# probsys/AutoGP.jl

Measured on AMD Instinct MI355X. Metric: particle_logpdf_evals_per_sec, higher is better.
Workload: dtype f64

## Files before the change

autogp.jl_amd/__init__.py:

```python
from .gp import (Node, LeafNode, BinaryOpNode, WhiteNoise, Constant, Linear, SquaredExponential,
                 GammaExponential, Periodic, Plus, Times, ChangePoint, unroll, encode, encode_batch, from_tuple,
                 split_kernel_sop, extract_kernel)
from .engine import (GPEngine, GPEngineMulti, shard_range, shard_plan, probe_lattice, logpdf_grad_batch_multi, predict_batch_multi, AGPError, PosDefException, load_library, LIB_PATH, EXPORTED_SYMBOLS,
                     compute_cov_matrix_vectorized, eval_cov, mvnormal_logpdf, MvNormal, quantile, infer_gp_sum, predict_proba,
                     predict_quantile, predict_quantile_multi, raw_components, predict_mvn_sum, predict_sum, predict_rand,
                     MixtureModel, predict_mvn, pack_series, series_call_args, SERIES_MAX_N)
from . import prior, schedule, dist, stream

__all__ = [n for n in dir() if not n.startswith("_")]
```

autogp.jl_amd/csrc/agp_common.hpp:

```cpp
#pragma once
#include <hip/hip_runtime.h>
#include <stdint.h>

namespace agp {

constexpr int NB = 128;
constexpr int NB2 = NB * NB;
constexpr int BS = 16;
constexpr int NSB = NB / BS;
constexpr int KB = 16;
constexpr int AGP_MAX_OPS_DEV = 256;
constexpr int LDS_STRIDE = 144;

enum : int { OP_WN = 0, OP_CONST = 1, OP_LIN = 2, OP_SE = 3, OP_GE = 4, OP_PER = 5,
             OP_PLUS = 6, OP_TIMES = 7, OP_CP = 8, OP_CP_SWAP = 9, OP_SEL = 10, OP_GE_TAB = 11,
             OP_LAG = 12 };
constexpr double LOGDT_ZERO = -1.0e8;

struct ProgHdr {
  int32_t op_off;
  int32_t prm_off;
  int32_t n_ops;
  int32_t n_cp;
  int32_t n_prm;
  int32_t flags;
  int32_t n_lag;
  int32_t lag_off;
};

struct LagTabHdr {
  int32_t op_off, n_ops, prm_off, pad_;
};

__host__ __device__ inline long long tile_off(int i, int j) {
  return ((long long)i * (i + 1) / 2 + j) * (long long)NB2;
}

typedef double d4 __attribute__((ext_vector_type(4)));
typedef double d2 __attribute__((ext_vector_type(2)));

}
```

autogp.jl_amd/csrc/agp_cov_kernel.hpp:

```cpp
#pragma once
#ifndef AGP_EXP_TABLE
#define AGP_EXP_TABLE 1
#endif
#include "agp_common.hpp"
#include "agp_args.hpp"
#include "agp_math.hpp"

namespace agp {

__device__ __forceinline__ int prm_count(int o) {
  return (o == OP_WN || o == OP_CONST || o == OP_SEL) ? 1 : (o == OP_SE || o == OP_CP || o == OP_CP_SWAP) ? 2
         : (o == OP_PLUS || o == OP_TIMES || o == OP_LAG) ? 0 : 3;
}

template <bool LAG = false, typename OpT>
__device__ __forceinline__ void cov_prologue(const double* __restrict__ tt, const uint8_t* __restrict__ code,
                                             int ti, int tj, const ProgHdr& h,
                                             const OpT* __restrict__ ops, const double* __restrict__ prm,
                                             double* tpt, double* sig, int tid,
                                             const double* __restrict__ lagtab = nullptr, int nt = 0,
                                             const int32_t* __restrict__ rank = nullptr, int lstride = 256, int* xrk = nullptr,
                                             bool copy_rank_tables = true, const CltArgs clt = CltArgs{}, int* cbl = nullptr) {
  const int g = (tid < NB) ? (ti * NB + tid) : (tj * NB + (tid - NB));
  const double tg = tt[g];
  if (LAG && h.n_lag > 0) {
    double* lag = sig + h.n_cp * 256;
    if (rank != nullptr) {
      if (clt.B != nullptr && copy_rank_tables) {
        const int odmin = clt.W > 0 ? (ti > tj ? (ti - tj) * NB - (NB - 1) : 0) : 0;
        const int woff = clt.W * odmin;
        for (int li = 0; li < h.n_lag; ++li) {
          const double* __restrict__ src = lagtab + (long long)(h.lag_off + li) * clt.gstride + woff;
          for (int i = tid; i < lstride; i += 256) lag[li * lstride + i] = src[i];
        }
        for (int i = tid; i < clt.nB; i += 256) cbl[i] = clt.B[odmin + i] - woff;
      } else {
        const double* __restrict__ src = lagtab + (long long)h.lag_off * lstride;
        if (copy_rank_tables)
          for (int i = tid; i < h.n_lag * lstride; i += 256) lag[i] = src[i];
      }
      xrk[tid] = rank[g];
    } else {
      const double* __restrict__ src = lagtab + ((long long)h.lag_off * nt + (ti - tj)) * 256 + tid;
      for (int li = 0; li < h.n_lag; ++li) lag[li * 256 + tid] = src[(long long)li * nt * 256];
    }
  }
  tpt[tid] = tg;
  __syncthreads();
  if (h.n_cp > 0) {
    const double t = tg;
    const int cd = code ? (int)code[g] : 0;
    int q = 0, c = 0;
    for (int ip = 0; ip < h.n_ops; ++ip) {
      const int o = __builtin_amdgcn_readfirstlane((int)ops[ip]);
      if (o == OP_CP || o == OP_CP_SWAP) {
        const double loc = prm[q], sc = prm[q + 1];
        sig[c * 256 + tid] = 0.5 * (1.0 + tanh((loc - t) / sc));
        ++c;
      } else if (o == OP_SEL) {
        const int id = (int)prm[q];
        sig[c * 256 + tid] = (cd == 0 || cd == id) ? 1.0 : 0.0;
        ++c;
      }
      q += prm_count(o);
    }
    __syncthreads();
  }
}

template <int E, int GEMODE>
__device__ __forceinline__ void eval_leaf(const int o, const double p0, const double p1, const double p2,
                                          const double* sg, const double* lg,
                                          const double (&tr)[E], const double (&tc)[E],
                                          const int (&ri)[E], const int (&ci)[E], const double (&lt)[E],
                                          const double* etab, double (&v)[E], const int* rk = nullptr, const int* cb = nullptr) {
  auto ex = [&](double x) { return (AGP_EXP_TABLE != 0) ? fm::exp_t(x, etab) : fm::exp_f(x); };
  if (o == OP_SEL) {
#pragma unroll
    for (int e = 0; e < E; ++e) v[e] = sg[ri[e]] * sg[ci[e]];
  } else if (o == OP_WN) {
#pragma unroll
    for (int e = 0; e < E; ++e) v[e] = (tr[e] == tc[e]) ? p0 : 0.0;
  } else if (o == OP_CONST) {
#pragma unroll
    for (int e = 0; e < E; ++e) v[e] = p0;
  } else if (o == OP_LIN) {
#pragma unroll
    for (int e = 0; e < E; ++e) v[e] = p1 + p2 * ((tr[e] - p0) * (tc[e] - p0));
  } else if ((GEMODE == 0 || GEMODE == 3) && (GEMODE == 3 || o == OP_LAG)) {
    if (cb != nullptr) {
#pragma unroll
      for (int e = 0; e < E; ++e) {
        const int d0 = rk[ri[e]] - rk[ci[e]], d = d0 < 0 ? -d0 : d0;
        v[e] = lg[(d & CLT_MASK) + cb[d >> CLT_SHIFT]];
      }
    } else if (rk != nullptr) {
#pragma unroll
      for (int e = 0; e < E; ++e) { const int d = rk[ri[e]] - rk[ci[e]]; v[e] = lg[d < 0 ? -d : d]; }
    } else {
      const double* lq_ = lg + (2 * NB - 1);
#pragma unroll
      for (int e = 0; e < E; ++e) v[e] = lq_[ri[e] - ci[e]];
    }
  } else if (GEMODE != 3) {
    double arg[E];
    const double amp = (o == OP_SE) ? p1 : p2;
    if (o == OP_SE) {
#pragma unroll
      for (int e = 0; e < E; ++e) {
        const double dx = tr[e] - tc[e];
        arg[e] = ((-0.5 * dx) * dx) * p0;
      }
    } else if (GEMODE != 2 && o == OP_GE) {
#pragma unroll
      for (int e = 0; e < E; ++e) arg[e] = -fm::pow_f(fabs(tr[e] - tc[e]) * p0, p1);
    } else if (GEMODE != 1 && (o == OP_GE_TAB || (GEMODE == 2 && o == OP_GE))) {
#pragma unroll
      for (int e = 0; e < E; ++e) arg[e] = -ex(p1 * (lt[e] - p0));
    } else {
#pragma unroll
      for (int e = 0; e < E; ++e) arg[e] = p0 * fm::sin2_f(p1 * fabs(tr[e] - tc[e]));
    }
#pragma unroll
    for (int e = 0; e < E; ++e) v[e] = amp * ex(arg[e]);
  }
}

template <int D, int E, int GEMODE = 0, typename OpT>
__device__ __forceinline__ void eval_program(const ProgHdr& h, const OpT* __restrict__ ops,
                                             const double* __restrict__ prm, const double* sig,
                                             const double (&tr)[E], const double (&tc)[E],
                                             const int (&ri)[E], const int (&ci)[E], const double (&lt)[E],
                                             double (&out)[E], const double* etab = nullptr, const double* lag = nullptr,
                                             const int* rk = nullptr, int lstride = 256, const int* cb = nullptr) {
  double st[D][E];
#pragma unroll
  for (int d = 0; d < D; ++d)
#pragma unroll
    for (int e = 0; e < E; ++e) st[d][e] = 0.0;

  int q = 0, cpi = 0, li = 0;
  for (int ip = 0; ip < h.n_ops; ++ip) {
    const int o = __builtin_amdgcn_readfirstlane((int)ops[ip]);
    if (o <= OP_PER || o >= OP_SEL) {
      const double p0 = prm[q], p1 = prm[q + 1], p2 = prm[q + 2];
      double v[E];
      eval_leaf<E, GEMODE>(o, p0, p1, p2, sig + cpi * 256, lag + li * lstride, tr, tc, ri, ci, lt, etab, v, rk, cb);
      if (o == OP_SEL) ++cpi;
      if (o == OP_LAG) ++li;
#pragma unroll
      for (int d = D - 1; d > 0; --d)
#pragma unroll
        for (int e = 0; e < E; ++e) st[d][e] = st[d - 1][e];
#pragma unroll
      for (int e = 0; e < E; ++e) st[0][e] = v[e];
    } else {
      if (o == OP_PLUS) {
#pragma unroll
        for (int e = 0; e < E; ++e) st[0][e] = st[1][e] + st[0][e];
      } else if (o == OP_TIMES) {
#pragma unroll
        for (int e = 0; e < E; ++e) st[0][e] = st[1][e] * st[0][e];
      } else {
        const double* sg = sig + cpi * 256;
#pragma unroll
        for (int e = 0; e < E; ++e) {
          const double si = sg[ri[e]];
          const double sj = sg[ci[e]];
          const double kl = (o == OP_CP) ? st[1][e] : st[0][e];
          const double kr = (o == OP_CP) ? st[0][e] : st[1][e];
          st[0][e] = (si * sj) * kl + ((1.0 - si) * (1.0 - sj)) * kr;
        }
        ++cpi;
      }
#pragma unroll
      for (int d = 1; d < D - 1; ++d)
#pragma unroll
        for (int e = 0; e < E; ++e) st[d][e] = st[d + 1][e];
    }
    q += prm_count(o);
  }
#pragma unroll
  for (int e = 0; e < E; ++e) out[e] = st[0][e];
}

__device__ __forceinline__ double cov_finalize(double v, int gi, int gj, int n1, int n1_pad, int m2, double noise) {
  const bool vi = (gi < n1) || (gi >= n1_pad && gi < n1_pad + m2);
  const bool vj = (gj < n1) || (gj >= n1_pad && gj < n1_pad + m2);
  double r = (vi && vj) ? v : 0.0;
  if (gi == gj) r = vi ? (r + noise) : 1.0;
  return r;
}
__device__ __forceinline__ double diag_noise(const double* noise, const double* noise_q, int p, int tk, int n1_pad) {
  const double* q = tk * NB < n1_pad ? noise : noise_q;
  return q != nullptr ? q[p] : 0.0;
}

#ifndef AGP_COV_E
#define AGP_COV_E 4
#endif
#ifndef AGP_COV_WGS
#define AGP_COV_WGS 4
#endif
template <int D>
__global__ __launch_bounds__(256, AGP_COV_WGS) void k_cov_tiles(CovArgs a) {
  constexpr int E = AGP_COV_E, CPP = E / 2;
  const int cpt = a.csplit == 4 ? 8 : 32;
  const int NPASS = cpt / CPP;
  extern __shared__ __attribute__((aligned(16))) double smem[];
  double* tpt = smem;
  double* sig = smem + 256;

  const int p = blockIdx.y + a.p_off;
  const int tix = blockIdx.x;
  int ti, tj;
  ti = (int)((sqrt(8.0 * (double)tix + 1.0) - 1.0) * 0.5);
  while (ti * (ti + 1) / 2 > tix) --ti;
  while ((ti + 1) * (ti + 2) / 2 <= tix) ++ti;
  tj = tix - ti * (ti + 1) / 2;
  if (a.i0 != nullptr && ti < a.i0[p]) return;
  if (a.skip_pred_offdiag && ti != tj && tj * NB >= a.n1_pad) return;
  if (a.pred_only && tj * NB < a.n1_pad) return;
  const int tid = threadIdx.x;
  const ProgHdr h = a.hdr[p];
  const uint8_t* __restrict__ ops = a.ops + h.op_off;
  const double* __restrict__ prm = a.prm + h.prm_off;
  const bool rankt = a.lagr != nullptr;
  const int lstride = rankt ? (a.clt.B != nullptr ? a.clt.gstride : a.lag_stride) : 256;
  int* xrk = reinterpret_cast<int*>(sig + h.n_cp * 256 + (rankt ? 0 : h.n_lag * 256));
  double* etab = reinterpret_cast<double*>(xrk) + (rankt ? 128 : 0);
  if (AGP_EXP_TABLE && tid < AGP_EXP_TAB_N) etab[tid] = fm::c_exp_tab[tid];
  cov_prologue<true>(a.tt, a.code, ti, tj, h, ops, prm, tpt, sig, tid, a.lagtab, a.nt, a.lagr, lstride, xrk, false);
  const double* lag = rankt ? a.lagtab + (long long)h.lag_off * lstride : sig + h.n_cp * 256;
  const int* rk = rankt ? xrk : nullptr;
  const int* cb = rankt ? a.clt.B : nullptr;

  const int rp = tid & 63;
  const int cb0 = a.csplit == 4 ? (int)blockIdx.z * 32 + (tid >> 6) * 8 : (tid >> 6) * 32;
  const int r0 = 2 * rp;
  const double tr0 = tpt[r0], tr1 = tpt[r0 + 1];
  const int gi0 = ti * NB + r0;
  const double noise = diag_noise(a.noise, a.noise_q, p, tj, a.n1_pad);
  double* __restrict__ T = a.A + (long long)(a.slot != nullptr ? a.slot[p] : p) * a.strideA + tile_off(ti, tj);

  const bool use_tab = (h.flags & 1) != 0;
  const double* __restrict__ ltile = a.logdt + tile_off(ti, tj);
  d2 ltn[CPP];
#pragma unroll
  for (int cc = 0; cc < CPP; ++cc) ltn[cc] = d2{0.0, 0.0};
  if (use_tab) {
#pragma unroll
    for (int cc = 0; cc < CPP; ++cc) ltn[cc] = *reinterpret_cast<const d2*>(ltile + (long long)(cb0 + cc) * NB + r0);
  }
  const bool one_node = h.n_ops == 1;
  const int op1 = one_node ? __builtin_amdgcn_readfirstlane((int)ops[0]) : -1;
  const double q0 = one_node ? prm[0] : 0.0, q1 = one_node ? prm[1] : 0.0, q2 = one_node ? prm[2] : 0.0;
  for (int pass = 0; pass < NPASS; ++pass) {
    const int c0 = cb0 + pass * CPP;
    double tr[E], tc[E], out[E], lt[E];
    int ri[E], ci[E];
#pragma unroll
    for (int cc = 0; cc < CPP; ++cc) { lt[2 * cc] = ltn[cc].x; lt[2 * cc + 1] = ltn[cc].y; }
    if (use_tab && pass + 1 < NPASS) {
#pragma unroll
      for (int cc = 0; cc < CPP; ++cc) ltn[cc] = *reinterpret_cast<const d2*>(ltile + (long long)(c0 + CPP + cc) * NB + r0);
    }
#pragma unroll
    for (int e = 0; e < E; ++e) {
      tr[e] = (e & 1) ? tr1 : tr0;
      tc[e] = tpt[NB + c0 + (e >> 1)];
      ri[e] = r0 + (e & 1);
      ci[e] = NB + c0 + (e >> 1);
    }
    if (one_node) eval_leaf<E, 0>(op1, q0, q1, q2, sig, lag, tr, tc, ri, ci, lt, etab, out, rk, cb);
    else eval_program<D, E, 0>(h, ops, prm, sig, tr, tc, ri, ci, lt, out, etab, lag, rk, lstride, cb);
#pragma unroll
    for (int cc = 0; cc < CPP; ++cc) {
      const int gj = tj * NB + c0 + cc;
      d2 o2;
      o2.x = cov_finalize(out[2 * cc], gi0, gj, a.n1, a.n1_pad, a.m2, noise);
      o2.y = cov_finalize(out[2 * cc + 1], gi0 + 1, gj, a.n1, a.n1_pad, a.m2, noise);
      *reinterpret_cast<d2*>(T + (long long)(c0 + cc) * NB + r0) = o2;
    }
  }
}

#ifdef AGP_KERNEL_TU_MAIN
__global__ __launch_bounds__(256) void k_lag_tables(LagArgs a) {
  const int t = blockIdx.y, bl = blockIdx.x, tid = threadIdx.x;
  __shared__ double etab[AGP_EXP_TAB_N];
  if (AGP_EXP_TABLE && tid < AGP_EXP_TAB_N) etab[tid] = fm::c_exp_tab[tid];
  __syncthreads();
  const LagTabHdr th = a.thdr[t];
  ProgHdr h = {};
  h.n_ops = th.n_ops;
  int g = a.full ? bl * 256 + tid : bl * NB + tid - (NB - 1);
  if (g < 0) g = -g;
  const bool live = a.full ? g < a.nt * NB : (tid < 2 * NB - 1 && g < a.nt * NB);
  const double tr[1] = {live ? a.tt[g] : 0.0}, tc[1] = {live ? a.tt[0] : 0.0}, lt[1] = {0.0};
  const int ri[1] = {0}, ci[1] = {NB};
  double out[1];
  eval_program<8, 1, 1>(h, a.tops + th.op_off, a.tprm + th.prm_off, nullptr, tr, tc, ri, ci, lt, out, etab);
  if (a.full) a.tab[(long long)t * a.stride + g] = out[0];
  else a.tab[((long long)t * a.nt + bl) * 256 + tid] = out[0];
}

__global__ __launch_bounds__(256) void k_logdt_tiles(const double* __restrict__ tt, double* __restrict__ T) {
  const int tix = blockIdx.x;
  int ti = (int)((sqrt(8.0 * (double)tix + 1.0) - 1.0) * 0.5);
  while (ti * (ti + 1) / 2 > tix) --ti;
  while ((ti + 1) * (ti + 2) / 2 <= tix) ++ti;
  const int tj = tix - ti * (ti + 1) / 2;
  double* __restrict__ out = T + tile_off(ti, tj);
  for (int e = threadIdx.x; e < NB2; e += 256) {
    const int r = e & (NB - 1), cidx = e >> 7;
    const double dt = fabs(tt[ti * NB + r] - tt[tj * NB + cidx]);
    out[e] = dt > 0.0 ? fm::log_f(dt) : LOGDT_ZERO;
  }
}

#endif

}
```

autogp.jl_amd/csrc/agp_engine.hip:

```cpp
#include "agp_host.hpp"

thread_local std::string g_err_noctx;

std::atomic<long long> HostProf::ns[HostProf::N];
std::atomic<long long> HostProf::cnt[HostProf::N];
const char* HostProf::names[HostProf::N] = {"coalesce: assemble", "dedup keys", "compile_batch", "grad classify + residency", "store lookup (grad)",
    "slot + buffers + staging", "launches (value)", "launches (grad)", "wait + copy back", "scatter results", "extend: keys + dedup",
    "extend: capacity + slots", "extend: compile", "extend: staging + launches", "extend: wait + register", "coalesce: hand back",
    "  of which: factor part", "  of which: gradient launches", "", "", "", "", "", ""};
int HostProf::enabled() {
  static int e = -1;
  if (e < 0) { const char* v = getenv("AGP_HOST_PROF"); e = (v && atoi(v) != 0) ? 1 : 0; }
  return e;
}
void HostProf::report() {
  if (enabled() <= 0) return;
  fprintf(stderr, "[AGP_HOST_PROF] stage                              calls     total ms    us / call\n");
  for (int i = 0; i < N; ++i) {
    const long long k = cnt[i].load(), t = ns[i].load();
    if (k > 0) fprintf(stderr, "[AGP_HOST_PROF] %-32s %8lld %12.2f %12.1f\n", names[i], k, (double)t / 1e6, (double)t / 1e3 / (double)k);
  }
}

int fail(agp_ctx* c, int code, const std::string& msg) {
// ... 79 lines not shown
  return s;
}

void release_slot(agp_ctx* c, Slot* s, bool async_done) {
  { std::lock_guard<std::mutex> g(c->mu); if (async_done) s->pending = true; else s->busy = false; }
  c->cv.notify_one();
}

struct CNode {
  int op; int left = -1, right = -1; double prm[3] = {0, 0, 0}; int need = 1;
  int prm_idx = 0;
};

struct Compiled {
  std::vector<uint8_t> ops;
  std::vector<double> prm;
  int n_cp = 0;
  int depth_need = 1;
  std::vector<CNode> nodes;
  int root = -1;
  int n_prm_caller = 0;
  bool uses_tab = false;
  int n_lag = 0;
  std::vector<LagTabHdr> thdr;
  std::vector<uint8_t> tops;
  std::vector<double> tprm;
};

constexpr int DYN_LDS_MAX_BYTES = 160 * 1024;
constexpr int COV_MAX_TABLES = (DYN_LDS_MAX_BYTES / 8 - 256 - 3 * AGP_MAX_OPS_DEV - AGP_MAX_OPS_DEV - 16) / 256;

int leaf_nprm(int op) {
  switch (op) {
    case OP_WN: case OP_CONST: case OP_SEL: return 1;
    case OP_SE: return 2;
    case OP_LIN: case OP_GE: case OP_PER: return 3;
    default: return -1;
  }
}

void classify(const std::vector<CNode>& nodes, int id, std::vector<char>& stat, std::vector<char>& heavy) {
  const CNode& nd = nodes[id];
  if (nd.left < 0) {
    stat[id] = nd.op == OP_WN || nd.op == OP_CONST || nd.op == OP_SE || nd.op == OP_GE || nd.op == OP_PER;
    heavy[id] = nd.op == OP_SE || nd.op == OP_GE || nd.op == OP_PER;
    return;
  }
  classify(nodes, nd.left, stat, heavy); classify(nodes, nd.right, stat, heavy);
  stat[id] = (nd.op == OP_PLUS || nd.op == OP_TIMES) && stat[nd.left] && stat[nd.right];
  heavy[id] = heavy[nd.left] || heavy[nd.right];
}

void emit(const std::vector<CNode>& nodes, int id, Compiled& out, bool ge_tab, bool lag = false,
          const std::vector<char>* stat = nullptr, const std::vector<char>* heavy = nullptr) {
  const CNode& nd = nodes[id];
  if (lag && stat && (*stat)[id] && (*heavy)[id]) {
    Compiled sub;
    emit(nodes, id, sub, false, false);
    LagTabHdr th;
    th.op_off = (int32_t)out.tops.size(); th.n_ops = (int32_t)sub.ops.size(); th.prm_off = (int32_t)out.tprm.size(); th.pad_ = 0;
    out.thdr.push_back(th);
    out.tops.insert(out.tops.end(), sub.ops.begin(), sub.ops.end());
    out.tprm.insert(out.tprm.end(), sub.prm.begin(), sub.prm.end());
    out.ops.push_back((uint8_t)OP_LAG);
    out.n_lag++;
    return;
  }
  if (nd.left < 0) {
    out.ops.push_back((uint8_t)nd.op);
    switch (nd.op) {
      case OP_WN: case OP_CONST: out.prm.push_back(nd.prm[0]); break;
      case OP_SEL: out.prm.push_back(nd.prm[0]); out.n_cp++; break;
      case OP_LIN: out.prm.insert(out.prm.end(), {nd.prm[0], nd.prm[1], nd.prm[2]}); break;
      case OP_SE: out.prm.insert(out.prm.end(), {1.0 / (nd.prm[0] * nd.prm[0]), nd.prm[1]}); break;
      case OP_GE:
        if (ge_tab) {
          out.ops.back() = (uint8_t)OP_GE_TAB;
          out.uses_tab = true;
          out.prm.insert(out.prm.end(), {std::log(nd.prm[0]), nd.prm[1], nd.prm[2]});
        } else {
          out.prm.insert(out.prm.end(), {1.0 / nd.prm[0], nd.prm[1], nd.prm[2]});
        }
        break;
      case OP_PER:
        out.prm.insert(out.prm.end(), {-2.0 / (nd.prm[0] * nd.prm[0]), M_PI / nd.prm[1], nd.prm[2]});
        break;
    }
    return;
  }
  const bool swap = nodes[nd.right].need > nodes[nd.left].need;
  emit(nodes, swap ? nd.right : nd.left, out, ge_tab, lag, stat, heavy);
  emit(nodes, swap ? nd.left : nd.right, out, ge_tab, lag, stat, heavy);
  if (nd.op == OP_CP) {
    out.ops.push_back((uint8_t)(swap ? OP_CP_SWAP : OP_CP));
    out.prm.push_back(nd.prm[0]);
    out.prm.push_back(nd.prm[1]);
    out.n_cp++;
  } else {
    out.ops.push_back((uint8_t)nd.op);
  }
}

const char* compile_program(const uint8_t* ops, int n_ops, const double* prm, int n_prm, Compiled& out,
                            bool allow_sel = false, bool ge_tab = false, bool lag = false) {
  if (n_ops <= 0 || n_ops > AGP_MAX_OPS) return "program length out of range";
  std::vector<CNode> nodes;
  nodes.reserve(n_ops);
  std::vector<int> stack;
  int ip = 0;
  for (int i = 0; i < n_ops; ++i) {
    const int op = ops[i];
    CNode nd; nd.op = op;
    if (op <= OP_PER || (allow_sel && op == OP_SEL)) {
      const int k = leaf_nprm(op);
      if (ip + k > n_prm) return "parameter array too short";
      for (int q = 0; q < k; ++q) nd.prm[q] = prm[ip + q];
      nd.prm_idx = ip;
      ip += k;
      nd.need = 1;
    } else if (op == OP_PLUS || op == OP_TIMES || op == OP_CP) {
      if (stack.size() < 2) return "postfix stack underflow";
      nd.right = stack.back(); stack.pop_back();
      nd.left = stack.back(); stack.pop_back();
      if (op == OP_CP) {
        if (ip + 2 > n_prm) return "parameter array too short";
        nd.prm[0] = prm[ip]; nd.prm[1] = prm[ip + 1]; nd.prm_idx = ip; ip += 2;
      }
      const int a = nodes[nd.left].need, b = nodes[nd.right].need;
      nd.need = (a == b) ? a + 1 : std::max(a, b);
    } else {
      return "unknown opcode";
    }
    nodes.push_back(nd);
    stack.push_back((int)nodes.size() - 1);
  }
  if (stack.size() != 1) return "postfix program does not reduce to one kernel";
  if (ip != n_prm) return "parameter count mismatch";
  out.depth_need = nodes[stack[0]].need;
  if (out.depth_need > 8) return "kernel tree needs an evaluation stack deeper than 8";
  if (lag) {
    std::vector<char> stat(nodes.size(), 0), heavy(nodes.size(), 0);
    classify(nodes, stack[0], stat, heavy);
    emit(nodes, stack[0], out, false, true, &stat, &heavy);
    if (out.n_cp + out.n_lag > COV_MAX_TABLES) {
      Compiled plain;
      emit(nodes, stack[0], plain, false, false);
      plain.depth_need = out.depth_need;
      out = plain;
    }
  } else {
    emit(nodes, stack[0], out, ge_tab, false);
  }
  if (out.n_cp > COV_MAX_TABLES) return "kernel tree needs more per-point LDS tables (ChangePoint nodes + component selectors) than fit 160 KiB";
  out.root = stack[0];
  out.n_prm_caller = n_prm;
  out.nodes.swap(nodes);
  return nullptr;
}

double op_cost_us(int op) {
  switch (op) {
    case OP_GE: return 36.0;
    case OP_GE_TAB: return 18.0;
    case OP_PER: return 12.0;
    case OP_SE: return 7.0;
    case OP_LIN: return 2.0;
    case OP_CP: case OP_CP_SWAP: return 2.0;
    case OP_LAG: return 2.0;
    default: return 0.6;
  }
}

int emit_grad(const std::vector<CNode>& nodes, int id, Batch& bt, int prm_base, int node_base) {
  const CNode& nd = nodes[id];
  int li = 0, ri = 0;
  if (nd.left >= 0) {
    const bool swap = nodes[nd.right].need > nodes[nd.left].need;
    if (swap) { ri = emit_grad(nodes, nd.right, bt, prm_base, node_base); li = emit_grad(nodes, nd.left, bt, prm_base, node_base); }
    else { li = emit_grad(nodes, nd.left, bt, prm_base, node_base); ri = emit_grad(nodes, nd.right, bt, prm_base, node_base); }
  }
  const int me = (int)bt.gops.size() - node_base;
  bt.gops.push_back((uint8_t)nd.op);
  bt.glc.push_back((uint8_t)li);
  bt.grc.push_back((uint8_t)ri);
  bt.gpoff.push_back((int32_t)bt.gprm.size() - prm_base);
  const int k = nd.left < 0 ? leaf_nprm(nd.op) : (nd.op == OP_CP ? 2 : 0);
  for (int q = 0; q < k; ++q) { bt.gprm.push_back(nd.prm[q]); bt.gmap.push_back(nd.prm_idx + q); }
  return me;
}

int compile_batch(agp_ctx* c, const Particles& pp, Batch& bt, const CompileOpts& o) {
  const int P = pp.P;
  std::vector<Compiled> cps(P);
  std::vector<double> cost(P, 0.0);
  for (int p = 0; p < P; ++p) {
    const char* e = compile_program(pp.program(p), pp.n_ops(p), pp.params(p), pp.n_prm(p), cps[p], o.allow_sel, o.ge_tab && !o.lag, o.lag);
    if (e) {
      char buf[256];
      snprintf(buf, sizeof buf, "particle %d: %s", p, e);
      return fail(c, AGP_ERR_PROGRAM, buf);
    }
    for (uint8_t o : cps[p].ops) cost[p] += op_cost_us(o);
  }
  const bool fuse_on = !o.never_fuse && (c->fuse_mode == 1 || (c->fuse_mode < 0 && (P >= 256 || o.fuse_hint)));
  const double fuse_limit = o.flow_limit ? (o.lag ? FLOW_LAG_FUSE_MAX_US : FLOW_FUSE_MAX_US) : (o.lag ? LAG_FUSE_MAX_US : FUSE_MAX_US);
  auto lag_ok = [&](int p) { bool direct = false; for (uint8_t o : cps[p].ops) direct |= (o == OP_SE || o == OP_GE || o == OP_PER || o == OP_GE_TAB); return !direct; };
  auto fusable = [&](int p) {
    if (o.lag) return fuse_on && cost[p] <= fuse_limit && lag_ok(p) && cps[p].n_cp + cps[p].n_lag * o.lag_units + o.rank_extra <= U_MAX_CP;
    return fuse_on && cost[p] <= fuse_limit && cps[p].n_cp <= U_MAX_CP;
  };
  bt.order.resize(P);
  for (int p = 0; p < P; ++p) bt.order[p] = p;
  std::stable_sort(bt.order.begin(), bt.order.end(), [&](int a, int b) {
    const bool fa = fusable(a), fb = fusable(b);
    if (fa != fb) return fa;
    return fa ? cost[a] > cost[b] : false;
  });
  bt.hdr.resize(P);
  for (int q = 0; q < P; ++q) {
    const Compiled& cp = cps[bt.order[q]];
    ProgHdr h;
    h.op_off = (int32_t)bt.ops.size();
    h.prm_off = (int32_t)bt.prm.size();
    h.n_ops = (int32_t)cp.ops.size();
    h.n_cp = cp.n_cp;
    h.n_prm = (int32_t)cp.prm.size();
    h.flags = cp.uses_tab ? 1 : 0;
    h.n_lag = cp.n_lag; h.lag_off = bt.n_lag_tables;
    bt.n_lag_tables += cp.n_lag;
    for (LagTabHdr th : cp.thdr) {
      th.op_off += (int32_t)bt.tops.size(); th.prm_off += (int32_t)bt.tprm.size();
      bt.thdr.push_back(th);
    }
    bt.tops.insert(bt.tops.end(), cp.tops.begin(), cp.tops.end());
    bt.tprm.insert(bt.tprm.end(), cp.tprm.begin(), cp.tprm.end());
    bt.hdr[q] = h;
    bt.ops.insert(bt.ops.end(), cp.ops.begin(), cp.ops.end());
    bt.prm.insert(bt.prm.end(), cp.prm.begin(), cp.prm.end());
    const int lds_units = cp.n_cp + cp.n_lag * o.lag_units + o.rank_extra;
    bt.max_cp = std::max(bt.max_cp, o.rank_extra > 0 ? cp.n_cp + 1 : lds_units);
    bt.max_depth = std::max(bt.max_depth, cp.depth_need);
    if (fusable(bt.order[q])) {
      bt.n_fused = q + 1;
      bt.max_cp_fused = std::max(bt.max_cp_fused, lds_units);
      bt.max_depth_fused = std::max(bt.max_depth_fused, cp.depth_need);
    }
  }
  if (o.want_grad) {
    bt.ghdr.resize(P);
    for (int q = 0; q < P; ++q) {
      const Compiled& cp = cps[bt.order[q]];
      GProgHdr g;
      g.node_off = (int32_t)bt.gops.size(); g.prm_off = (int32_t)bt.gprm.size();
      emit_grad(cp.nodes, cp.root, bt, g.prm_off, g.node_off);
      g.n_ops = (int32_t)bt.gops.size() - g.node_off; g.n_prm = (int32_t)bt.gprm.size() - g.prm_off;
      g.n_cp = cp.n_cp; g.flags = 0;
      for (int i2 = g.node_off; i2 < (int)bt.gops.size(); ++i2) if (bt.gops[i2] == OP_GE) g.flags = 1;
      bt.ghdr[q] = g;
      bt.g_max_nodes = std::max(bt.g_max_nodes, g.n_ops);
      bt.g_max_prm = std::max(bt.g_max_prm, g.n_prm);
      bt.g_max_cp = std::max(bt.g_max_cp, g.n_cp);
    }
    bt.gprm.push_back(0.0); bt.gprm.push_back(0.0); bt.gprm.push_back(0.0);
  }
  while (bt.ops.size() % 4) bt.ops.push_back(0);
  bt.prm.push_back(0.0); bt.prm.push_back(0.0);
  while (bt.tops.size() % 4) bt.tops.push_back(0);
  bt.tprm.push_back(0.0); bt.tprm.push_back(0.0); bt.tprm.push_back(0.0);
  return AGP_OK;
}


int64_t ws_limit_bytes(agp_ctx* c) {
  if (c->ws_limit > 0) return c->ws_limit;
  int64_t lim = (int64_t)(c->total_mem * 0.55);
  const int64_t cap = 96LL << 30;
  lim = std::min(lim, cap);
  const int64_t store = (int64_t)c->store.footprint.load(std::memory_order_relaxed);
  if (store > 0) lim = std::max<int64_t>(std::min<int64_t>(lim, (int64_t)(c->total_mem * 0.92) - store), 1LL << 30);
  return lim;
}

struct Prof {
  agp_ctx* c; Slot* s; hipStream_t st; bool on; size_t next = 0;
  std::vector<std::pair<int, std::pair<size_t, size_t>>> spans;
  hipEvent_t ev() {
    if (next >= s->events.size()) {
      hipEvent_t e; (void)hipEventCreate(&e); s->events.push_back(e);
    }
    return s->events[next++];
  }
  size_t mark() { return mark(st); }
  size_t mark(hipStream_t q) {
    if (!on) return 0;
    size_t i = next; hipEvent_t e = ev(); (void)hipEventRecord(e, q); return i;
  }
  void span(int kind, size_t a, size_t b) { if (on) spans.push_back({kind, {a, b}}); }
  void collect(double* acc) {
    if (!on) return;
    std::vector<double> u, t;
// ... 399 lines not shown
      {
        std::lock_guard<std::mutex> g(c->mu);
        c->n_toeplitz_value += n_done;
        if (via_store) {
          if (c->schur_keys.size() > 32768) c->schur_keys.clear();
          for (size_t b2 = 0; b2 < part[1].size(); ++b2)
            if (sT.info[b2] == 0) {
              const int p = part[1][b2];
              c->schur_keys.insert(particle_key(pp, p));
            }
        }
      }
      const int rcR = dense(refused);
      if (rcR) return rcR;
      return AGP_OK;
    }
  }

  if (tl_dense_via_store && !go && h_out_lp && h_out_info) {
    TlClear plain(tl_dense_via_store);
    return extend_impl(c, n, pp, h_out_lp, h_out_info);
  }
  Batch bt;
  std::vector<std::vector<int32_t>> pls;
  pls.reserve(64);
  const bool ge_tab = c->logdt_ok;
  const bool flow_hint = n > 0 && use_flow(c, P, (int)((n + NB - 1) / NB));
  const bool lag = allow_lag && c->lag_enable && c->lag_ok && c->lag_contig && !go && n > 0 && n == c->n_max;
  const int rank_units = (int)((c->n_lat + 255) / 256);
  bool lagr = !lag && allow_lag && c->lag_rank_enable && c->lag_enable && c->lag_ok && n > 0 && rank_units <= LAG_LDS_MAX_UNITS;
  const bool clt = !lag && !lagr && allow_lag && c->lag_rank_enable && c->lag_enable && c->clt_ok && n > 0;
  const int clt_wunits = clt ? (int)(((int64_t)c->clt_W * c->n_max + 255) / 256) : 0;
  const bool cltw = clt && clt_wunits <= LAG_LDS_MAX_UNITS;
  const bool clts = clt && !cltw && !go && n == c->n_max;
  const bool rankm = lagr || cltw || clts;
  const int tab_units = cltw ? clt_wunits : clts ? c->clt_W : rank_units;
  const int tab_gstride = (cltw || clts) ? c->clt_gstride : rank_units * 256;
  const int clt_nB = cltw ? (int)((c->n_max + 1) & ~(int64_t)1) : clts ? 256 : 0;
  const int rank_extra = (cltw || clts) ? (256 + clt_nB + 511) / 512 : lagr ? 1 : 0;
  const bool sorted = lag || clts;
  HostProf hp_cb(2);
  CompileOpts co;
  co.want_grad = go != nullptr; co.ge_tab = ge_tab; co.fuse_hint = co.flow_limit = flow_hint;
  co.lag = lag || rankm; co.lag_units = rankm ? tab_units : 1; co.rank_extra = rank_extra;
  int rc = compile_batch(c, pp, bt, co);
  hp_cb.stop();
  if (rc) return rc;
  HostProf hp_cls(3);
  if (lagr) { std::lock_guard<std::mutex> g(c->mu); ++c->n_lag_rank_sweeps; }
  if (cltw || clts) { std::lock_guard<std::mutex> g(c->mu); ++c->n_clt_sweeps; }
  if (go && bt.g_max_nodes > 64) return fail(c, AGP_ERR_PROGRAM, "gradient supports kernel trees of up to 64 nodes");
  if (go && n > 23040) return fail(c, AGP_ERR_ARG, "gradient sweeps address a particle's packed matrix with 32-bit byte offsets: n <= 23040");
  if (lag) { std::lock_guard<std::mutex> g(c->mu); ++c->n_lag_sweeps; }
  int32_t toep_rank0 = 0;
  bool any_toep_sweep = false;
  std::vector<int32_t> toep_retry;
  if (go && n > 0 && c->grad_lagdom && c->lag_enable && c->lag_ok && c->n_lat <= LAGDOM_MAX_BINS) {
    int64_t n_cov = 0, n_sum = 0;
    const bool use_fft = c->lag_contig && c->grad_fft && c->d_fft_tw != nullptr && 2 * c->n_max <= FFT_N && n > GRAD_FFT_MIN_N;
    bool use_toep = c->lag_contig && !tl_no_toep && c->grad_fft >= 2 && c->d_fft_tw != nullptr && 2 * c->n_max <= FFT_N && n >= GRAD_TOEP_MIN_N && (int64_t)c->h_rank.size() >= n;
    if (use_toep) {
      int32_t lo = c->h_rank[0], hi = c->h_rank[0];
      for (int64_t i = 1; i < n; ++i) { lo = std::min(lo, c->h_rank[(size_t)i]); hi = std::max(hi, c->h_rank[(size_t)i]); }
      use_toep = (int64_t)hi - lo + 1 == n;
      toep_rank0 = lo;
    }
    for (int q = 0; q < P; ++q) {
      GProgHdr& g = bt.ghdr[q];
      if (g.n_cp > 0 || g.n_ops > 64) continue;
      uint8_t stat[64], cov[64], deg[64];
      for (int i = 0; i < g.n_ops; ++i) {
        const int o = bt.gops[g.node_off + i], li = bt.glc[g.node_off + i], ri = bt.grc[g.node_off + i];
        if (o == OP_PLUS || o == OP_TIMES) {
          stat[i] = stat[li] && stat[ri];
          cov[i] = stat[i] || (o == OP_PLUS && cov[li] && cov[ri]);
          deg[i] = (uint8_t)std::min(100, o == OP_PLUS ? std::max<int>(deg[li], deg[ri]) : deg[li] + deg[ri]);
        } else {
          stat[i] = (o == OP_SE || o == OP_GE || o == OP_PER || o == OP_CONST || o == OP_WN);
          cov[i] = stat[i] || o == OP_LIN;
          deg[i] = o == OP_LIN ? 1 : 0;
        }
      }
      if (g.n_ops > 0 && cov[g.n_ops - 1]) { g.flags |= GFLAG_LAGDOM | (use_toep ? GFLAG_LAGTOEP : use_fft ? GFLAG_LAGFFT : 0); ++n_cov; ++n_sum; }
      else if (g.n_ops > 0 && c->grad_lagdom >= 2 && deg[g.n_ops - 1] >= 1 && deg[g.n_ops - 1] <= 3 &&
               (2 * deg[g.n_ops - 1] + 1) * c->n_lat + 8 <= NB2) {
        g.flags |= GFLAG_LAGPOLY | ((int)deg[g.n_ops - 1] << GFLAG_POLY_DEG_SHIFT); ++n_cov;
      }
    }
    const bool store_live = c->factor_cache && c->store.n_slots > 0;
    std::vector<char> resident((size_t)P, 0);
    int64_t n_struct = n_sum;
    if (store_live && c->toeplitz && use_toep && n_sum > 0) {
      std::lock_guard<std::mutex> g(c->store.mu);
      agp_ctx::FactorStore& fs = c->store;
      for (int q = 0; q < P; ++q) {
        if (!(bt.ghdr[q].flags & GFLAG_LAGTOEP)) continue;
        const int p = bt.order[q];
        auto it = fs.index.find(particle_key(pp, p));
        if (it != fs.index.end() && fs.n_cached[(size_t)it->second] == n && fs.info_h[(size_t)it->second] == 0) { resident[(size_t)q] = 1; --n_struct; }
      }
    }
    bool sticky = false;
    if (store_live && c->toeplitz && use_toep && n_struct > 0) {
      std::lock_guard<std::mutex> g(c->mu);
      if (!c->schur_keys.empty())
        for (int q = 0; q < P && !sticky; ++q) {
// ... 183 lines not shown
      up.add(s->grc.p, bt.grc.data(), bt.grc.size());
      up.add(s->gpoff.p, bt.gpoff.data(), sizeof(int32_t) * bt.gpoff.size());
      up.add(s->gprm.p, bt.gprm.data(), sizeof(double) * bt.gprm.size());
      up.add(s->gmap.p, bt.gmap.data(), sizeof(int32_t) * bt.gmap.size());
      up.add(s->goff.p, goff_sorted.data(), sizeof(int32_t) * P);
      HIPCHK(c, up.flush(s->h_stage2, s->up_blob2, st));
    }
    if ((lag || rankm) && bt.n_lag_tables > 0) {
      LagArgs la = {};
      la.tt = (cltw || clts) ? c->d_clt_tt : lagr ? c->d_ts_lat : c->d_ts_s;
      lpl.point(la, dstage);
      if (rankm) {
        HIPCHK(c, s->lagtab.ensure(sizeof(double) * (size_t)bt.n_lag_tables * tab_gstride));
        la.tab = s->lagtab.as<double>(); la.nt = lagr ? (int)((c->n_lat + NB - 1) / NB) : tab_gstride / NB; la.full = 1; la.stride = tab_gstride;
        launch_lag_tables(st, la, tab_gstride / 256, bt.n_lag_tables);
      } else {
        HIPCHK(c, s->lagtab.ensure(sizeof(double) * (size_t)bt.n_lag_tables * nt * 256));
        la.tab = s->lagtab.as<double>(); la.nt = nt;
        launch_lag_tables(st, la, nt, bt.n_lag_tables);
      }
      HIPCHK(c, hipGetLastError());
    }
    size_t ev_h2d = pf.mark();
    HostProf hp_fac(16);
    pf.span(7, ev_begin, ev_h2d);

    for (int p0 = 0; p0 < P; p0 += chunk) {
      const int Pc = std::min(chunk, P - p0);
      {
        const int g0 = 0, Pg = Pc;
        hipStream_t q = st;
        launch_init_vec(q, n_pad, Pg, s->vec.as<double>() + (size_t)g0 * n_pad, sorted ? c->d_xs_s : c->d_xs, (const double*)nullptr, (int)n, s->info.as<int>() + g0, s->ready.as<int>() + g0);
        CovArgs cv = {};
        cv.tt = sorted ? c->d_ts_s : c->d_ts; cv.n1 = (int)n; cv.n1_pad = n_pad; cv.m2 = 0; cv.nt = nt;
        cv.hdr = d_hdr + p0 + g0; cv.ops = d_ops; cv.prm = d_prm;
        cv.noise = d_noise + p0 + g0; cv.A = s->A.as<double>() + (size_t)g0 * strideA;
        cv.strideA = strideA; cv.P = Pg; cv.logdt = (ge_tab && !lag && !rankm) ? c->d_logdt : nullptr;
        cv.lagtab = (lag || rankm) ? s->lagtab.as<double>() : nullptr;
        cv.lagr = lagr ? c->d_rank : cltw ? c->d_clt_key : clts ? c->d_clt_key_s : nullptr; cv.lag_stride = tab_units * 256;
        if (cltw || clts) { cv.clt.B = c->d_clt_B; cv.clt.W = clts ? c->clt_W : 0; cv.clt.nB = clt_nB; cv.clt.gstride = tab_gstride; }
        int i0min = 0;
        if (n_hit > 0) {
          launch_gather(c, q, Pg, nt, cv.A, strideA, s->W.as<double>() + (size_t)g0 * NSB * 256 * wsteps, wsteps,
                        s->vec.as<double>() + (size_t)g0 * n_pad, n_pad, s->partial.as<double>() + (size_t)g0 * 2 * nt, nt,
                        d_src + p0 + g0, s->ready.as<int>() + g0, false);
          cv.i0 = d_i0 + p0 + g0;
          i0min = nt;
          for (int r = 0; r < Pg; ++r) i0min = std::min(i0min, (int)i0v[(size_t)p0 + g0 + r]);
        }
        const int nf = std::max(0, std::min(Pg, bt.n_fused - p0 - g0));
        const int dcov = nf > 0 ? bt.max_depth_fused : 0;
        size_t e0 = pf.mark(q);
        cv.p_off = nf;
        if (!(n_hit > 0 && i0min == nt)) HIPCHK(c, launch_cov(q, cv, ntiles, Pg - nf, bt.max_cp, bt.max_depth));
        size_t e1 = pf.mark(q);
        pf.span(1, e0, e1);

        CholArgs ca = {};
        ca.A = cv.A; ca.strideA = strideA; ca.W = s->W.as<double>() + (size_t)g0 * NSB * 256 * wsteps;
        ca.wsteps = wsteps;
        ca.vec = s->vec.as<double>() + (size_t)g0 * n_pad; ca.ldv = n_pad;
        ca.partial = s->partial.as<double>() + (size_t)g0 * 2 * nt;
        ca.info = s->info.as<int>() + g0; ca.P = Pg; ca.nt = nt; ca.k = 0; ca.nt1 = nt;
        set_cov(ca, cv);
        ca.lag = (lag || rankm) ? 1 : 0;
        ca.n_fused = nf;
        ca.ready = s->ready.as<int>() + g0;
        ca.i0 = cv.i0;
        if (n_hit > 0 && i0min == nt) {
        } else if (use_flow(c, ca.P, nt)) {
          const int ntri = nt * (nt + 1) / 2;
          ca.tflag = s->tflag.as<int>() + (size_t)g0 * ntri; ca.ntri = ntri;
          ca.qnext = s->flowq.as<int>();
          {
            size_t items = 0;
            for (int x = 0; x < 8; ++x) items += (size_t)((Pg - x + 7) / 8) * ntri;
            ca.trace = (c->d_flow_trace && items <= c->flow_trace_items && P <= chunk) ? c->d_flow_trace : nullptr;
          }
          if (n_hit > 0)
            launch_init_flow_flags(q, Pg, ca.tflag, ntri, ntri, (const int*)nullptr, ca.i0);
          else
            HIPCHK(c, hipMemsetAsync(ca.tflag, 0, sizeof(int) * (size_t)Pg * ntri, q));
          HIPCHK(c, hipMemsetAsync(ca.qnext, 0, sizeof(int) * 8, q));
          size_t f0 = pf.mark(q);
          launch_flow(dcov, 2 * c->n_cu, q, ca);
          size_t f1 = pf.mark(q);
          pf.span(2, f0, f1);
          if (c->profiling) tacc[5] += 1;
          HIPCHK(c, hipGetLastError());
        } else if (n_hit > 0) {
          HIPCHK(c, run_factor_extend(q, ca, dcov, use_split_diag(c, ca.P), i0min));
        } else {
          HIPCHK(c, run_factor(q, ca, nt, dcov, c->profiling ? &pf : nullptr, c->profiling ? &tacc[5] : nullptr, use_split_diag(c, ca.P),
                               use_right_looking(c, ca.P), HYBRID_BLOCKS));
        }

        size_t e2 = pf.mark(q);
        launch_finish_logpdf(q, ca.partial, ca.info, nt, Pg, (int)n, d_map + p0 + g0, d_lp, d_info_out);
        size_t e3 = pf.mark(q);
        pf.span(4, e2, e3);
        HIPCHK(c, hipGetLastError());
        if (go) {
          hp_fac.stop();
          HostProf hp_gl(17);
          GradArgs ga = {};
          ga.A = cv.A; ga.Z = s->Z.as<double>() + (size_t)g0 * strideA; ga.strideA = strideA; ga.W = ca.W;
          ga.beta = ca.vec; ga.alpha = s->alpha.as<double>() + (size_t)g0 * n_pad; ga.ldv = n_pad;
// ... 407 lines not shown
        for (int k = 1; k <= LATTICE_MAX_DIV && !lattice; ++k) {
          const double h0 = dmin / (double)k;
          if ((t1 - t0) / h0 > (double)(max_lat - 1) || (table_bound && 2.0 * ((t1 - t0) / h0) > (double)n_max * (double)n_max)) break;
          bool ok = true;
          for (int64_t i = 0; ok && i < n_max; ++i) {
            const double q = (tss[(size_t)i] - t0) / h0, g = std::nearbyint(q);
            ok = std::fabs(q - g) <= 1e-3;
            lat[(size_t)i] = (int64_t)g;
          }
          if (!ok || lat.back() <= 0) continue;
          const double h1 = (t1 - t0) / (double)lat.back();
          for (int64_t i = 0; ok && i < n_max; ++i) ok = std::fabs(tss[(size_t)i] - (t0 + (double)lat[(size_t)i] * h1)) <= tol_l;
          if (ok) { lattice = true; hl = h1; n_lat = lat.back() + 1; dmin_lat = dmin; }
        }
      }
    }
    if (regular) { lat.resize((size_t)n_max); for (int64_t i = 0; i < n_max; ++i) lat[(size_t)i] = i; }
    lf.kind = regular ? 1 : lattice ? 2 : 0;
    lf.h = hl; lf.dmin = regular ? h : dmin_lat; lf.n_lat = n_lat;
    if (lf.kind) lf.index.swap(lat);
  }
  return lf;
}

struct CompactFit {
  bool ok = false;
  int64_t W = 0;
  LatticeFit lat;
  std::vector<int64_t> base;
};
static CompactFit fit_compact(const std::vector<double>& tss, double lag_tol_h, double hint_h = 0.0) {
  CompactFit cf;
  const int64_t n_max = (int64_t)tss.size();
  if (n_max < 3 || n_max > CLT_MAX_N) return cf;
  cf.lat = fit_lattice(tss, lag_tol_h, true, hint_h, CLT_MAX_LAT, false);
  if (cf.lat.kind != 2 || cf.lat.n_lat > CLT_MAX_LAT) return cf;
  const std::vector<int64_t>& gl = cf.lat.index;
  std::vector<int64_t> top((size_t)n_max, 0);
  cf.base.assign((size_t)n_max, INT64_MAX);
  cf.base[0] = 0;
  for (int64_t i = 0; i < n_max; ++i)
    for (int64_t j = i + 1; j < n_max; ++j) {
      const int64_t lagv = gl[(size_t)j] - gl[(size_t)i];
      int64_t& b = cf.base[(size_t)(j - i)]; int64_t& tp = top[(size_t)(j - i)];
      if (lagv < b) b = lagv;
      if (lagv > tp) tp = lagv;
    }
  cf.W = 1;
  for (int64_t od = 1; od < n_max; ++od) cf.W = std::max(cf.W, top[(size_t)od] - cf.base[(size_t)od] + 1);
  cf.ok = cf.W <= CLT_MAX_W;
  return cf;
}

int agp_probe_lattice(const double* ts, int64_t n, int32_t* kind, int64_t* n_lattice, double* spacing, int64_t* index_out) {
  if (n < 0 || (n > 0 && !ts)) return AGP_ERR_ARG;
  for (int64_t i = 0; i < n; ++i)
    if (!std::isfinite(ts[i])) {
      if (kind) *kind = 0;
      if (n_lattice) *n_lattice = 0;
      if (spacing) *spacing = 0.0;
      if (index_out) for (int64_t j = 0; j < n; ++j) index_out[j] = -1;
      return AGP_OK;
    }
  try {
    std::vector<int64_t> perm((size_t)n);
    for (int64_t i = 0; i < n; ++i) perm[(size_t)i] = i;
    std::stable_sort(perm.begin(), perm.end(), [&](int64_t a, int64_t b) { return ts[a] < ts[b]; });
    std::vector<double> tss((size_t)n);
    for (int64_t i = 0; i < n; ++i) tss[(size_t)i] = ts[perm[(size_t)i]];
    LatticeFit lf = fit_lattice(tss, 1e-11, true);
    if (lf.kind == 0) {
      CompactFit cf = fit_compact(tss, 1e-11);
      if (cf.ok) { lf = std::move(cf.lat); lf.kind = 3; }
    }
    if (kind) *kind = lf.kind;
    if (n_lattice) *n_lattice = lf.kind ? lf.n_lat : 0;
    if (spacing) *spacing = lf.kind ? lf.h : 0.0;
    if (index_out) for (int64_t i = 0; i < n; ++i) index_out[perm[(size_t)i]] = lf.kind ? lf.index[(size_t)i] : -1;
  } catch (...) { return AGP_ERR_HOST; }
  return AGP_OK;
}

static int set_data_body(agp_ctx* c, const double* ts, const double* xs, int64_t n_max, const std::vector<uint8_t>* keep = nullptr) {
  if (!c) return fail(nullptr, AGP_ERR_ARG, "null context");
  if (n_max < 0 || (n_max > 0 && (!ts || !xs))) return fail(c, AGP_ERR_ARG, "bad data arguments");
  HIPCHK(c, hipSetDevice(c->device));
  HIPCHK(c, hipDeviceSynchronize());
  {
    std::lock_guard<std::mutex> g(c->store.mu);
    const bool prefix = c->n_max > 0 && n_max >= c->n_max &&
                        std::memcmp(ts, c->h_ts.data(), sizeof(double) * (size_t)c->n_max) == 0 &&
                        std::memcmp(xs, c->h_xs.data(), sizeof(double) * (size_t)c->n_max) == 0;
    if (!prefix && !keep) {
      c->store.forget(); c->store.ghost_clear();
      { std::lock_guard<std::mutex> gk(c->mu); c->schur_keys.clear(); }
      std::lock_guard<std::mutex> q(c->qmu);
      c->caller_ids.clear(); c->n_callers = 0;
    }
  }
  const bool lag_was = c->lag_ok, contig_was = c->lag_contig;
  const bool clt_was = c->clt_ok;
  const bool small_was = c->n_max > 0 && (c->n_max + NB - 1) / NB <= 2;
  const double clt_h_was = c->clt_h, clt_t0_was = c->clt_t0;
  const std::vector<double> tlat_was = c->h_ts_lat;
  const double grid_h_was = c->grid_h;
  const double t0_was = c->h_ts_sorted.empty() ? std::nan("") : c->h_ts_sorted.front();
// ... 459 lines not shown
```

autogp.jl_amd/csrc/agp_host.hpp:

```cpp
#pragma once
#include "../../include/autogp_hip.h"
#include "agp_common.hpp"
#include "agp_args.hpp"
#include "agp_launch.hpp"
#include "agp_comm.hpp"
#include "agp_particles.hpp"

#include <algorithm>
#include <atomic>
#include <cmath>
#include <chrono>
#include <condition_variable>
#include <cstdio>
#include <cstdlib>
#include <cstring>
#include <functional>
#include <memory>
#include <mutex>
#include <new>
#include <exception>
#include <string>
#include <system_error>
#include <thread>
#include <deque>
// ... 197 lines not shown
  int n_cu = 256;
  bool profiling = false;
  int64_t pred_reused = 0, pred_factored = 0;
  int64_t grad_reused = 0, grad_factored = 0;
  int factor_cache = 1;
  int remove_update = 1;
  int64_t rm_updated = 0, rm_dropped = 0, rm_rows = 0, rm_panels = 0;
  int predict_reuse = 1;
  int dedup = 1;
  int64_t n_particles_seen = 0, n_particles_run = 0;
  int64_t n_mix_passes = 0, n_mix_chunks = 0;
  int split_diag = -1;
  int ge_table = 1;
  double* d_ts_s = nullptr;
  double* d_xs_s = nullptr;
  int lag_rank_enable = 1;
  int64_t n_lag_rank_sweeps = 0;
  int32_t* d_rank = nullptr;
  double t_ref = 0.0;
  double grid_h = 0.0, grid_mid = 0.0;
  int grad_fft = 2;
  double* d_fft_tw = nullptr;
  int grad_lagdom = 2;
  double poly_mmax = 1.0;
  int64_t n_lagdom_particles = 0;
  int64_t n_struct_pred = 0;
  int64_t n_struct_grad = 0;
  int grad_struct = 1;
  int64_t n_toep_particles = 0;
  bool lag_ok = false;
  bool lag_contig = false;
  double lat_tol_abs = 0.0;
  int64_t n_lat = 0;
  std::unordered_set<std::string> schur_keys;
  int ref_arith = 0;
  int lattice_enable = 1;
  bool clt_ok = false;
  int clt_W = 0;
  double clt_h = 0.0, clt_t0 = 0.0;
  int32_t* d_clt_key = nullptr;
  int32_t* d_clt_key_s = nullptr;
  int32_t* d_clt_B = nullptr;
  double* d_clt_tt = nullptr;
  int clt_gstride = 0;
  int64_t clt_n_lat = 0;
  int64_t n_clt_sweeps = 0;
  std::vector<double> h_ts_lat;
  double* d_ts_lat = nullptr;
  int toeplitz = 0;
  int64_t n_toeplitz_value = 0;
  int lag_enable = 1;
  double lag_tol_h = 1e-11;
  int64_t n_lag_sweeps = 0;
  double* d_logdt = nullptr;
  size_t logdt_cap = 0;
  bool logdt_ok = false;
  int right_looking = -1;
  int flow = -1;
  long long* d_flow_trace = nullptr;
  size_t flow_trace_items = 0;
  PoisonCtl poison;
  int fuse_mode = -1;
  double timing[16] = {0, 0, 0, 0, 0, 0, 0, 0, 0, 0, 0, 0, 0, 0, 0, 0};
  std::vector<double> upd_ms, trsm_ms;
  std::mutex qmu;
  std::condition_variable qcv_leader;
  bool leader_gathering = false;
  long long arrivals = 0;
  int batch_prev = 0;
  double last_sweep_us = 0.0;
  std::vector<LpRequest*> queue;
  std::unordered_set<std::thread::id> caller_ids;
  std::atomic<int> n_callers{0};
  std::atomic<int> inflight{0};
  bool leader_active = false;
  int coalesce_us = 2000;
  int batch_hint = 1;
  long long n_coalesced_calls = 0, n_coalesced_batches = 0;
  double co_wait_us = 0.0, co_value_us = 0.0, co_grad_us = 0.0, co_handback_us = 0.0;
  std::vector<double> h_xs;
  struct FactorStore {
    std::mutex mu;
    int nt_cap = 0;
    std::atomic<int> n_slots{0};
    long long strideA = 0;
    DevBuf A{Fill::values}, W{Fill::values}, vec{Fill::values}, partial{Fill::values};
    DevBuf info{Fill::never}, ready{Fill::never}, tflag{Fill::never}, flowq{Fill::never};
    DevBuf Z{Fill::values}, zalpha{Fill::values}, zdinv{Fill::values};
    std::vector<int32_t> zrows;
    void z_release() { Z.release(); zalpha.release(); zdinv.release(); std::fill(zrows.begin(), zrows.end(), 0); }
    std::vector<std::string> key;
    std::vector<int64_t> n_cached;
    std::vector<uint64_t> stamp;
    std::vector<int32_t> info_h;
    std::vector<uint8_t> used;
    std::vector<uint64_t> born;
    std::vector<uint64_t> slot_caller;
    std::unordered_map<uint64_t, int> caller_slot;
    std::unordered_set<std::string> ghost;
    std::deque<std::string> ghost_fifo;
    int64_t evicted_before_reuse = 0;
    void ghost_add(const std::string& k) {
      if (ghost.insert(k).second) ghost_fifo.push_back(k);
      while (ghost_fifo.size() > 8192) { ghost.erase(ghost_fifo.front()); ghost_fifo.pop_front(); }
    }
    void ghost_probe(const std::string& k) { if (!ghost.empty() && ghost.erase(k)) ++evicted_before_reuse; }
// ... 7 lines not shown
    size_t failed_bytes = 0;
    void forget() { failed_bytes = 0; index.clear(); std::fill(key.begin(), key.end(), std::string()); std::fill(n_cached.begin(), n_cached.end(), 0); std::fill(zrows.begin(), zrows.end(), 0); std::fill(used.begin(), used.end(), 0); std::fill(born.begin(), born.end(), 0); std::fill(slot_caller.begin(), slot_caller.end(), 0); caller_slot.clear(); }
    void release() { A.release(); W.release(); vec.release(); partial.release(); info.release(); ready.release(); tflag.release(); flowq.release(); z_release(); zrows.clear(); n_slots = 0; nt_cap = 0; footprint = 0; failed_bytes = 0; forget(); key.clear(); n_cached.clear(); stamp.clear(); info_h.clear(); used.clear(); born.clear(); slot_caller.clear(); caller_slot.clear(); }
  } store;
  ncclComm_t comm = nullptr;
  int comm_rank = 0, comm_size = 1;
  hipStream_t comm_stream = nullptr;
  std::mutex comm_mu;
  DevBuf comm_in{Fill::values}, comm_out{Fill::values}, comm_all{Fill::values};
  bool async_fault = false;
  int claimed_waits = 0;
  struct Worker {
    std::thread th;
    std::mutex mu;
    std::condition_variable cv;
    std::function<void()> job;
    bool has_job = false, done = true, stop = false;
  };
  Worker* worker = nullptr;
  std::mutex multi_mu;
};

int fail(agp_ctx* c, int code, const std::string& msg);

#define HIPCHK(ctx, expr)                                                                   \
  do {                                                                                      \
    hipError_t e_ = (expr);                                                                 \
    if (e_ != hipSuccess) {                                                                 \
      char buf_[512];                                                                       \
      snprintf(buf_, sizeof buf_, "HIP error %d (%s) at %s:%d: %s", (int)e_,                \
               hipGetErrorString(e_), __FILE__, __LINE__, #expr);                           \
      return fail(ctx, AGP_ERR_HIP, buf_);                                                  \
    }                                                                                       \
  } while (0)

Slot* acquire_slot(agp_ctx* c);
void release_slot(agp_ctx* c, Slot* s, bool async_done = false);
struct SlotGuard {
  agp_ctx* c; Slot* s;
  bool async_done = false;
  SlotGuard(agp_ctx* c_) : c(c_), s(acquire_slot(c_)) {}
  ~SlotGuard() { release(); }
  void release() { if (s) { release_slot(c, s, async_done); s = nullptr; } }
};

struct Batch {
  std::vector<ProgHdr> hdr;
  std::vector<uint8_t> ops;
  std::vector<double> prm;
  std::vector<int32_t> order;
  int n_fused = 0;
  int max_cp = 0;
  int max_depth = 1;
  int max_cp_fused = 0, max_depth_fused = 1;
  int n_lag_tables = 0;
  std::vector<LagTabHdr> thdr;
  std::vector<uint8_t> tops;
  std::vector<double> tprm;
  std::vector<GProgHdr> ghdr;
  std::vector<uint8_t> gops, glc, grc;
  std::vector<int32_t> gpoff, gmap;
  std::vector<double> gprm;
  int g_max_nodes = 0, g_max_prm = 0, g_max_cp = 0;
};

struct CompileOpts {
  bool allow_sel = false, want_grad = false, ge_tab = false;
  bool fuse_hint = false;
  bool flow_limit = false;
  bool lag = false;
  int lag_units = 1;
  int rank_extra = 0;
  bool never_fuse = false;
};
int compile_batch(agp_ctx* c, const Particles& pp, Batch& bt, const CompileOpts& o = {});

inline size_t align16(size_t x) { return (x + 15) & ~(size_t)15; }

struct LagProgLayout {
  const Batch& bt;
  size_t o_thdr, o_tprm, o_tops, end;
  explicit LagProgLayout(const Batch& b, size_t base = 0)
      : bt(b), o_thdr(align16(base)), o_tprm(align16(o_thdr + sizeof(LagTabHdr) * b.thdr.size())),
        o_tops(align16(o_tprm + sizeof(double) * b.tprm.size())), end(align16(o_tops + b.tops.size() + 4)) {}
  void pack(char* h) const {
    if (bt.thdr.empty()) return;
    std::memcpy(h + o_thdr, bt.thdr.data(), sizeof(LagTabHdr) * bt.thdr.size());
    std::memcpy(h + o_tprm, bt.tprm.data(), sizeof(double) * bt.tprm.size());
    std::memcpy(h + o_tops, bt.tops.data(), bt.tops.size());
  }
  hipError_t upload(PinnedUploads& up, DevBuf& dev) const {
    std::vector<char> h(end, 0);
    pack(h.data());
    const hipError_t e = dev.ensure(end);
    if (e == hipSuccess) up.add(dev.p, h.data(), end);
    return e;
  }
  void point(LagArgs& la, const void* dev) const {
    const char* d = static_cast<const char*>(dev);
    la.thdr = reinterpret_cast<const LagTabHdr*>(d + o_thdr);
    la.tprm = reinterpret_cast<const double*>(d + o_tprm);
    la.tops = reinterpret_cast<const uint8_t*>(d + o_tops);
    la.n_tables = bt.n_lag_tables;
  }
};

constexpr double FUSE_MAX_US = 25.0, FLOW_FUSE_MAX_US = 70.0, FLOW_LAG_FUSE_MAX_US = 10.0, LAG_FUSE_MAX_US = 3.0;
// ... 174 lines not shown
```

autogp.jl_amd/csrc/agp_kernels.hip:

```cpp
#define AGP_KERNEL_TU_MAIN 1
#include "agp_launch.hpp"
#include "agp_cov_kernel.hpp"
#include "agp_chol_kernel.hpp"
#include "agp_toep_kernel.hpp"
#include "agp_quantile_kernel.hpp"
#include "agp_sum_kernel.hpp"
#include "agp_sample_kernel.hpp"
#include "agp_mixmom_kernel.hpp"
#include "agp_comm.hpp"

namespace agp {

__global__ void k_compact_shards(const double* __restrict__ padded, int mx, int P, int n_ranks, double* __restrict__ out) {
  const int g = blockIdx.x * blockDim.x + threadIdx.x;
  if (g >= P) return;
  const int base = P / n_ranks, rem = P % n_ranks;
  int r = (g < rem * (base + 1)) ? g / (base + 1) : rem + (base > 0 ? (g - rem * (base + 1)) / base : 0);
  int lo, hi;
  shard_range(P, r, n_ranks, &lo, &hi);
  out[g] = padded[(long long)r * mx + (g - lo)];
}


constexpr int DYN_LDS_MAX_BYTES_K = 160 * 1024;

static hipError_t raise_dynamic_lds(const void* f) {
  hipFuncAttributes fa;
  hipError_t e = hipFuncGetAttributes(&fa, f);
  if (e == hipSuccess) e = hipFuncSetAttribute(f, hipFuncAttributeMaxDynamicSharedMemorySize, DYN_LDS_MAX_BYTES_K - (int)fa.sharedSizeBytes);
  return e;
}

hipError_t kernels_init() {
  const void* fns[] = {reinterpret_cast<const void*>(&k_cov_tiles<4>), reinterpret_cast<const void*>(&k_cov_tiles<8>)};
  for (const void* f : fns) { hipError_t e = raise_dynamic_lds(f); if (e != hipSuccess) return e; }
  return hipSuccess;
}

hipError_t launch_cov(hipStream_t st, const CovArgs& ca, int ntiles, int P, int max_cp, int depth) {
  if (ntiles <= 0 || P <= 0) return hipSuccess;
  const size_t lds = (256 + (size_t)max_cp * 256 + AGP_EXP_TAB_N) * sizeof(double);
  CovArgs cs = ca;
  cs.csplit = ((long long)ntiles * P < 4096) ? 4 : 1;
  dim3 grid(ntiles, P, cs.csplit), block(256);
  if (depth <= 4) hipLaunchKernelGGL(k_cov_tiles<4>, grid, block, lds, st, cs);
  else hipLaunchKernelGGL(k_cov_tiles<8>, grid, block, lds, st, cs);
  return hipGetLastError();
}

void launch_lag_tables(hipStream_t st, const LagArgs& la, int units, int n_tables) {
  hipLaunchKernelGGL(k_lag_tables, dim3(units, n_tables), dim3(256), 0, st, la);
}

hipError_t launch_toep_logpdf(hipStream_t st, const ToepArgs& ta) {
  if (ta.n > 256 * TOEP_MAX_R) return hipErrorInvalidValue;
  if (ta.pacc != nullptr) {
    if (ta.nj > 256 * TOEP_MAX_R || ta.n > 2048 || ta.Lcols == nullptr) return hipErrorInvalidValue;
    hipLaunchKernelGGL((k_toep_logpdf<8, true, true, 512>), dim3(ta.P), dim3(512), sizeof(double) * (8 * 512 + 16), st, ta);
    hipLaunchKernelGGL(k_toep_back<8>, dim3(ta.P), dim3(256), 0, st, ta);
  } else if (ta.Lcols != nullptr) {
    if (ta.n > 2048) return hipErrorInvalidValue;
    hipLaunchKernelGGL((k_toep_logpdf<8, true>), dim3(ta.P), dim3(256), sizeof(double) * (8 * 256 + 16), st, ta);
    hipLaunchKernelGGL(k_toep_back<8>, dim3(ta.P), dim3(256), 0, st, ta);
  } else if (ta.n <= 2048) {
    hipLaunchKernelGGL(k_toep_logpdf<8>, dim3(ta.P), dim3(256), sizeof(double) * (8 * 256 + 16), st, ta);
  } else {
    hipLaunchKernelGGL(k_toep_logpdf<TOEP_MAX_R>, dim3(ta.P), dim3(256), sizeof(double) * (TOEP_MAX_R * 256 + 16), st, ta);
  }
  return hipGetLastError();
}

void launch_logdt_tiles(hipStream_t st, unsigned ntiles, const double* ts, double* out) {
  hipLaunchKernelGGL(k_logdt_tiles, dim3(ntiles), dim3(256), 0, st, ts, out);
}

template <bool FACTOR, bool INTRSM, int DM>
static void launch_update(int dcov, int grid, hipStream_t st, const CholArgs& ca) {
  constexpr bool CAN_GM = FACTOR && INTRSM;
  const int gm = (CAN_GM && dcov > 0) ? (ca.lag ? 2 : (ca.logdt != nullptr ? 1 : 0)) : 0;
  const dim3 g(grid), b(256);
  if (dcov == 0) hipLaunchKernelGGL((k_chol_update<FACTOR, 0, INTRSM, DM>), g, b, 0, st, ca);
  else if (dcov <= 4) {
    if (gm == 2) hipLaunchKernelGGL((k_chol_update<FACTOR, 4, INTRSM, DM, CAN_GM ? 2 : 0>), g, b, 0, st, ca);
    else if (gm == 1) hipLaunchKernelGGL((k_chol_update<FACTOR, 4, INTRSM, DM, CAN_GM ? 1 : 0>), g, b, 0, st, ca);
    else hipLaunchKernelGGL((k_chol_update<FACTOR, 4, INTRSM, DM>), g, b, 0, st, ca);
  } else {
    if (gm == 2) hipLaunchKernelGGL((k_chol_update<FACTOR, 8, INTRSM, DM, CAN_GM ? 2 : 0>), g, b, 0, st, ca);
    else if (gm == 1) hipLaunchKernelGGL((k_chol_update<FACTOR, 8, INTRSM, DM, CAN_GM ? 1 : 0>), g, b, 0, st, ca);
    else hipLaunchKernelGGL((k_chol_update<FACTOR, 8, INTRSM, DM>), g, b, 0, st, ca);
  }
}
void launch_update_factor(int dcov, int grid, hipStream_t st, const CholArgs& ca) { launch_update<true, true, 0>(dcov, grid, st, ca); }
void launch_update_subdiag(int dcov, int grid, hipStream_t st, const CholArgs& ca) { launch_update<true, true, 2>(dcov, grid, st, ca); }
void launch_update_schur(int dcov, int grid, hipStream_t st, const CholArgs& ca) { launch_update<false, false, 0>(dcov, grid, st, ca); }
// ... 98 lines not shown
```

autogp.jl_amd/csrc/agp_launch.hpp:

```cpp
#pragma once
#include "agp_args.hpp"

namespace agp {

hipError_t kernels_init();
hipError_t launch_cov(hipStream_t st, const CovArgs& ca, int ntiles, int P, int max_cp, int depth);
void launch_lag_tables(hipStream_t st, const LagArgs& la, int units, int n_tables);
hipError_t launch_toep_logpdf(hipStream_t st, const ToepArgs& ta);
void launch_logdt_tiles(hipStream_t st, unsigned ntiles, const double* ts, double* out);
void launch_update_factor(int dcov, int grid, hipStream_t st, const CholArgs& ca);
void launch_update_subdiag(int dcov, int grid, hipStream_t st, const CholArgs& ca);
void launch_update_schur(int dcov, int grid, hipStream_t st, const CholArgs& ca);
void launch_diag(int dcov, int grid, hipStream_t st, const CholArgs& ca);
void launch_flow(int dcov, int n_wg, hipStream_t st, const CholArgs& ca);
void launch_trsm(int grid, hipStream_t st, const CholArgs& ca);
void launch_init_vec(hipStream_t st, int ldv, int P, double* vec, const double* xs, const double* mu1, int n1, int* info, int* ready);
void launch_finish_logpdf(hipStream_t st, const double* partial, const int* info, int nt, int P, int n, const int* map,
                          double* out_logpdf, int* out_info, const int* slot = nullptr, int ntp = 0);
void launch_init_query_vec(hipStream_t st, int P, double* vec, int ldv, int off, int m, const double* y, const double* mu2);
void launch_finish_pred_logpdf(hipStream_t st, const double* partial, const int* info, int nt1, int nt, int P, int m, int n,
                               int n1_pad, const int* map, double* out_logpdf, int* out_info);
void launch_init_extend(hipStream_t st, int U, double* vec, int ldv, int n_pad, const double* xs, int n, const int* slot,
                        const int* i0, int* info, int* ready);
void launch_init_flow_flags(hipStream_t st, int P, int* tflag, int ntri_stride, int ntri, const int* slot, const int* i0);
void launch_gather_factor(hipStream_t st, int gx, int P, const GatherArgs& ga);
void launch_copy_rows(hipStream_t st, int gx, int rows, double* dst, long long dpitch, const double* src, long long spitch, long long width);
void launch_poison_rows(hipStream_t st, int gx, int U, int nbuf, const PoisonRowsArgs& a);
void launch_scatter_uploads(hipStream_t st, const void* blob, int n_items, int slices);
void launch_expand_rep(hipStream_t st, int P, const double* lp, const int32_t* rep, double* out);
void launch_pred_extract(hipStream_t st, long long nel, int P, const PredArgs& pa);
void launch_unpack_dense(hipStream_t st, const double* A, int n, int lower_only, double* out);
void launch_pack_dense(hipStream_t st, const double* K, int n, int nt, long long n_packed, double* A);
void launch_compact_shards(hipStream_t st, const double* padded, int mx, int P, int n_ranks, double* out);
void launch_mfma_probe(const double* A, const double* B, double* D);
void launch_math_probe(int which, const double* x, const double* g, double* y, int n);
void launch_mfma_peak(int nblk, double* out, long long* cycles, int iters, int mode);
void launch_mixture_pack(hipStream_t st, const double* means, const double* vars, int P, int Pp, int m, double* cm, double* cs);
void launch_mixture_quantile(hipStream_t st, const double* cm, const double* cs, const double* cw, int Pp, int m, const double* q,
                             int nq, double tol, long long max_iter, double* out_x, int32_t* out_conv, int32_t* out_iters);
void launch_sum_readout(hipStream_t st, int P, const SumReadArgs& a);
void launch_philox_normals(hipStream_t st, const SampleNormArgs& a);
void launch_pred_sample(hipStream_t st, int n_groups, int nt2, const SampleReadArgs& a);
void launch_mixmom_chunk(hipStream_t st, const MixMomArgs& a);
void launch_mixmom_finish(hipStream_t st, const MixMomArgs& a);

hipError_t kernels_init_grad();
void launch_trtri_chain(hipStream_t st, int grid, const GradArgs& ga);
void launch_zspec(hipStream_t st, int nt, int P, const GradArgs& ga);
void launch_toep_solve(hipStream_t st, int P, size_t lds, const GradArgs& ga);
void launch_kinv_tiles(hipStream_t st, int grid, const GradArgs& ga);
hipError_t launch_grad_contract(int maxs, hipStream_t st, const GradArgs& ga, int ntiles, int P, size_t lds);
void launch_lag_grad(hipStream_t st, int P, size_t lds, const GradArgs& ga);
void launch_grad_finish(hipStream_t st, int P, const GradArgs& ga);

hipError_t kernels_init_series();
hipError_t launch_series_logpdf(hipStream_t st, const SeriesArgs& sa, int grid, int depth, size_t lds_bytes);
hipError_t launch_series_logpdf_grad(hipStream_t st, const SeriesGradArgs& sa, int grid, int depth, int tape, size_t lds_bytes);
hipError_t launch_series_probe(hipStream_t st, const SeriesProbeArgs& sa, int grid, size_t lds_bytes);

// ... 2 lines not shown
```

autogp.jl_amd/csrc/agp_predict.hip:

```cpp
#include "agp_host.hpp"
#include "agp_ndtri.hpp"
#ifdef AGP_EXPERIMENTS
#include "experiments/agp_experiments_abi.h"
#include "experiments/agp_experiments.hpp"
#endif


#ifdef AGP_EXPERIMENTS
template <int VAR>
static void launch_variant(hipStream_t st, int grid, const CholArgs& ca) {
  hipLaunchKernelGGL(k_gemm_variant<VAR>, dim3(grid), dim3(256), 0, st, ca);
}
#endif
namespace {

struct PredLattice {
  bool on = false;
  int R = 0, rank_units = 1;
  std::vector<int32_t> rank;
  std::vector<double> tl;
};
constexpr int64_t PRED_MAX_LAGS = LAG_LDS_MAX_UNITS * 256;

void predict_lattice(agp_ctx* c, int64_t n, const double* ts_pred, int64_t m, PredLattice& pl) {
// ... 241 lines not shown
  }
  if (n_hit > 0) {
    HIPCHK(c, s->stage.ensure(sizeof(int32_t) * 3 * (size_t)P));
    int32_t* d = s->stage.as<int32_t>();
    up.add(d, src_slot.data(), sizeof(int32_t) * P);
    up.add(d + P, i0v.data(), sizeof(int32_t) * P);
    if (zstore) { up.add(d + 2 * P, zi0v.data(), sizeof(int32_t) * P); d_zi0 = d + 2 * P; }
    d_src = d; d_i0 = d + P;
  }
  if (!lagr) {
    HIPCHK(c, up.flush(s->h_stage, s->up_blob, st));
  } else {
    std::vector<int32_t> rankF;
    if (diag_path) {
      rankF.assign((size_t)ntot, 0);
      std::copy(pl->rank.begin(), pl->rank.begin() + n1_pad, rankF.begin());
      for (int64_t g = 0; g < mJ; ++g) rankF[(size_t)n1_pad + g] = pl->rank[(size_t)n1_pad + fq[(size_t)g]];
    }
    if (const int rc = flush_lattice(c, s, st, up, bt, *pl, diag_path ? rankF : pl->rank)) return rc;
  }

  if (ro) HIPCHK(c, hipMemsetAsync(s->out_info.p, 0x7f, sizeof(int32_t) * (size_t)P, st));
  const double* h_mean = nullptr; const double* h_var = nullptr; const double* h_alpha = nullptr; const double* h_dinv = nullptr;
  const double* h_x = nullptr;
  for (int p0 = 0; p0 < P; p0 += chunk) {
    const int Pc = std::min(chunk, P - p0);
    {
      const size_t nm = (size_t)std::max<int64_t>(1, mJ) * Pc, nd = diag_path ? (size_t)ntot * Pc : 0;
      HIPCHK(c, s->h_out.ensure(sizeof(double) * (2 * nm + 2 * nd + nm * nq)));
      double* hz = static_cast<double*>(s->h_out.p);
      h_mean = hz; h_var = hz + nm; h_alpha = hz + 2 * nm; h_dinv = hz + 2 * nm + nd; h_x = hz + 2 * nm + 2 * nd;
    }
    launch_init_vec(st, ntot, Pc, s->vec.as<double>(), c->d_xs, (mean_train && n > 0) ? s->mu1.as<double>() : (const double*)nullptr, (int)n, s->info.as<int>() + p0, s->ready.as<int>() + p0);
    if (n_hit > 0) {
      launch_gather(c, st, Pc, nt1, s->A.as<double>(), strideA, s->W.as<double>(), nt1, s->vec.as<double>(), ntot, nullptr, 0,
                    d_src + p0, s->ready.as<int>() + p0);
      HIPCHK(c, hipGetLastError());
      if (p0 + chunk >= P && !zstore) {
        HIPCHK(c, hipStreamSynchronize(st));
        store_lk.unlock();
      }
    }
    CovArgs cv = {};
    cv.tt = s->tt.as<double>(); cv.n1 = (int)n; cv.n1_pad = n1_pad; cv.m2 = (int)mJ; cv.nt = nt;
    cv.hdr = s->hdr.as<ProgHdr>() + p0; cv.ops = s->ops.as<uint8_t>(); cv.prm = s->prm.as<double>();
    cv.noise = s->noise.as<double>() + p0; cv.A = s->A.as<double>(); cv.strideA = strideA; cv.P = Pc;
    cv.code = pred_code ? s->code.as<uint8_t>() : nullptr;
    if (lagr) { cv.lagtab = s->lagtab.as<double>(); cv.lagr = s->pl_rank.as<int32_t>(); cv.lag_stride = pl->rank_units * 256; }
    const int nf = std::max(0, std::min(Pc, bt.n_fused - p0));
    const int dcov = nf > 0 ? bt.max_depth_fused : 0;
    cv.p_off = nf;
    cv.skip_pred_offdiag = want_cov ? 0 : 1;
    cv.i0 = n_hit > 0 ? d_i0 + p0 : nullptr;
    HIPCHK(c, launch_cov(st, cv, ntiles, Pc - nf, bt.max_cp, bt.max_depth));

    CholArgs ca = {};
    ca.A = s->A.as<double>(); ca.strideA = strideA; ca.W = s->W.as<double>();
    ca.vec = s->vec.as<double>(); ca.ldv = ntot; ca.partial = s->partial.as<double>();
    ca.info = s->info.as<int>() + p0; ca.P = Pc; ca.nt = nt; ca.k = 0; ca.nt1 = nt1;
    set_cov(ca, cv);
    ca.lag = lagr ? 1 : 0;
    ca.n_fused = nf;
    ca.ready = s->ready.as<int>() + p0;
    if (n_hit > 0 || diag_path) ca.wsteps = nt1;
    if (n_hit > 0) ca.i0 = d_i0 + p0;
    if (nt1 > 0 && (sum ? c->flow != 0 : use_flow(c, Pc, nt, nt1))) {
      if (const int rc = launch_joint_flow(c, s, st, ca, dcov, nt1)) return rc;
    } else if (n_hit > 0) {
      int i0min = nt1;
      for (int q = 0; q < Pc; ++q) i0min = std::min(i0min, (int)i0v[(size_t)p0 + q]);
      HIPCHK(c, run_factor_extend(st, ca, dcov, use_split_diag(c, ca.P), i0min, nt1));
    } else {
      HIPCHK(c, run_factor(st, ca, nt1, dcov, nullptr, nullptr, use_split_diag(c, ca.P)));
    }
    if (diag_path) {
      GradArgs ga = {};
      ga.A = s->A.as<double>(); ga.strideA = strideA; ga.Z = s->Z.as<double>(); ga.strideZ = strideZ; ga.W = s->W.as<double>();
      ga.beta = s->vec.as<double>(); ga.alpha = s->alpha.as<double>(); ga.dinv = s->gpart.as<double>(); ga.ldv = ntot;
      ga.P = Pc; ga.nt = nt1; ga.n = (int)n;
      if (zstore) {
        agp_ctx::FactorStore& fs = c->store;
        ga.lslot = d_src + p0; ga.Lsrc = fs.A.as<double>(); ga.Lstride = fs.strideA; ga.Wsrc = fs.W.as<double>(); ga.Wnt = fs.nt_cap;
        ga.Zsrc = fs.Z.as<double>(); ga.Zstride = fs.strideA; ga.zi0 = d_zi0 + p0;
        ga.zalpha = fs.zalpha.as<double>(); ga.zdinv = fs.zdinv.as<double>(); ga.zld = (long long)fs.nt_cap * NB;
        ga.zfull = (int)(n / NB);
      }
      if (zstore && c->poison.active()) {
        agp_ctx::FactorStore& fs = c->store;
        PoisonRowsArgs pa = {};
        double* bases[3] = {fs.Z.as<double>(), fs.zalpha.as<double>(), fs.zdinv.as<double>()};
        const long long pitch[3] = {fs.strideA, (long long)fs.nt_cap * NB, (long long)fs.nt_cap * NB};
        const long long unit[3] = {NB2, NB, NB};
        for (int b = 0; b < 3; ++b) { pa.base[b] = bases[b]; pa.pitch[b] = pitch[b]; pa.unit[b] = unit[b]; pa.tri[b] = b == 0; }
        pa.nt_cap = fs.nt_cap; pa.slot = d_src + p0; pa.i0 = d_zi0 + p0;
        launch_poison_rows(st, 256, Pc, 3, pa);
        HIPCHK(c, hipGetLastError());
        for (int q = p0; q < p0 + Pc; ++q) {
          if (src_slot[(size_t)q] < 0 || zi0v[(size_t)q] < 0) continue;
          const long long r0 = std::min<long long>(zi0v[(size_t)q], fs.nt_cap);
          c->poison.count(sizeof(double) * (size_t)((fs.strideA - r0 * (r0 + 1) / 2 * NB2) + 2 * (fs.nt_cap - r0) * NB));
        }
      }
      if (zstore) zguard.armed = true;
      launch_trtri_chain(st, 8 * ((Pc + 7) / 8) * nt1, ga);
      if (zstore && p0 + chunk >= P) {
        HIPCHK(c, hipGetLastError());
        HIPCHK(c, hipStreamSynchronize(st));
        for (int q = 0; q < P; ++q) if (src_slot[(size_t)q] >= 0) c->store.zrows[(size_t)src_slot[(size_t)q]] = (int32_t)(n / NB);
        zguard.armed = false;
        store_lk.unlock();
      }
      HIPCHK(c, hipGetLastError());
      HIPCHK(c, hipMemcpyAsync(const_cast<double*>(h_alpha), s->alpha.p, sizeof(double) * ntot * Pc, hipMemcpyDeviceToHost, st));
      HIPCHK(c, hipMemcpyAsync(const_cast<double*>(h_dinv), s->gpart.p, sizeof(double) * ntot * Pc, hipMemcpyDeviceToHost, st));
    }
    if (mJ > 0) {
      ca.schur_diag_only = want_cov ? 0 : 1;
      const int T = want_cov ? nt2 * (nt2 + 1) / 2 : nt2;
      const int Pg = (Pc + 7) / 8;
      int dcov_s = dcov;
      if (lagr && nf > 0) {
        CovArgs cp = cv;
        cp.p_off = 0; cp.pred_only = 1; cp.i0 = nullptr;
        HIPCHK(c, launch_cov(st, cp, ntiles, nf, bt.max_cp, bt.max_depth));
        ca.n_fused = 0; dcov_s = 0;
      }
      launch_update_schur(dcov_s, 8 * Pg * T, st, ca);
    }
    if (mJ > 0) {
    PredArgs pa = {};
    pa.A = s->A.as<double>(); pa.strideA = strideA; pa.vec = s->vec.as<double>(); pa.ldv = ntot;
    pa.mu2 = mean_pred ? s->mu2.as<double>() : nullptr; pa.noise_pred = s->noise_pred.as<double>() + p0;
    pa.nt1 = nt1; pa.n1_pad = n1_pad; pa.m = (int)mJ; pa.P = Pc;
    pa.diag_add = diag_add ? s->diag_add.as<double>() : nullptr;
    pa.np_code = sum ? s->code.as<uint8_t>() + n1_pad : nullptr;
    pa.out_mean = s->pred_mean.as<double>(); pa.out_var = s->pred_var.as<double>();
    pa.out_cov = want_cov ? s->pred_cov.as<double>() : nullptr;
    const long long nel = want_cov ? (long long)mJ * mJ : (long long)mJ;
    launch_pred_extract(st, nel, Pc, pa);
    HIPCHK(c, hipGetLastError());
    if (mix)
      if (const int rc = mix_chunk(c, s, st, *mix, p0, Pc, pa.out_mean, pa.out_var, pa.out_cov)) return rc;
    if (ro) {
      SumReadArgs ra = {};
      ra.mean = s->pred_mean.as<double>(); ra.var = s->pred_var.as<double>(); ra.m = (int)mJ; ra.p_rows = (int)sum->p_rows;
      ra.slope = sum->slope; ra.intercept = sum->intercept; ra.shift = sum->intercept / sum->slope;
      ra.ivar = 1.0 / (sum->slope * sum->slope);
      ra.z = s->sum_z.as<double>(); ra.nq = nq; ra.x = s->sum_x.as<double>(); ra.bad = s->out_info.as<int32_t>() + p0;
      launch_sum_readout(st, Pc, ra);
      HIPCHK(c, hipGetLastError());
      if (nq > 0)
        HIPCHK(c, hipMemcpyAsync(const_cast<double*>(h_x), s->sum_x.p, sizeof(double) * mJ * nq * Pc, hipMemcpyDeviceToHost, st));
    }
    if (!mix) HIPCHK(c, hipMemcpyAsync(const_cast<double*>(h_mean), s->pred_mean.p, sizeof(double) * mJ * Pc, hipMemcpyDeviceToHost, st));
    if (!ro && !mix) HIPCHK(c, hipMemcpyAsync(const_cast<double*>(h_var), s->pred_var.p, sizeof(double) * mJ * Pc, hipMemcpyDeviceToHost, st));
    }
    HIPCHK(c, hipStreamSynchronize(st));
    for (int q = 0; q < Pc && !mix; ++q) {
      const size_t o = (size_t)bt.order[p0 + q];
      if (diag_path) {
        double* om = out_mean + o * m; double* ov = out_var + o * m;
        for (int64_t g = 0; g < mJ; ++g) { om[fq[(size_t)g]] = h_mean[(size_t)q * mJ + g]; ov[fq[(size_t)g]] = h_var[(size_t)q * mJ + g]; }
        const double s2 = noise_sorted[(size_t)p0 + q], np2 = npred[(size_t)p0 + q];
        const double* al = h_alpha + (size_t)q * ntot; const double* dv = h_dinv + (size_t)q * ntot;
        for (size_t d = 0; d < dq.size(); ++d) {
          const int32_t j = dq[d], i = di[d];
          const double ymu = c->h_xs[(size_t)i] - (mean_train ? mean_train[i] : 0.0);
          om[j] = (mean_pred ? mean_pred[j] : 0.0) + ymu - s2 * al[i];
          ov[j] = s2 - s2 * s2 * dv[i] + np2 + (diag_add ? diag_add[j] : 0.0);
        }
        continue;
      }
      std::memcpy(out_mean + o * m, h_mean + (size_t)q * m, sizeof(double) * m);
      if (!ro) std::memcpy(out_var + o * m, h_var + (size_t)q * m, sizeof(double) * m);
      if (nq > 0) std::memcpy(sum->out_x + o * m * nq, h_x + (size_t)q * m * nq, sizeof(double) * m * nq);
      if (out_cov)
        HIPCHK(c, hipMemcpyAsync(out_cov + o * m * m, s->pred_cov.as<double>() + (size_t)q * m * m,
// ... 27 lines not shown
int predict_logpdf_core(agp_ctx* c, const PredQuery& q, const double* y_pred, const Particles& pp, Batch& bt, double* out_lp,
                        int32_t* out_info, const PredLattice* pl, JointHooks* hooks) {
  const int64_t n = q.n, m = q.m;
  const int P = pp.P;
  const double* mean_train = q.mean_train; const double* mean_pred = q.mean_pred;
  const int n1_pad = round_up(n, NB), m_pad = round_up(m, NB);
  const bool lagr = pl != nullptr && pl->on;
  const int nt1 = n1_pad / NB, nt = nt1 + m_pad / NB;
  const int ntot = n1_pad + m_pad;
  const int ntiles = nt * (nt + 1) / 2;
  const long long strideA = (long long)ntiles * NB2;
  const int chunk = (int)std::max<int64_t>(1, std::min<int64_t>(P, ws_limit_bytes(c) / (strideA * 8)));

  SlotGuard sg(c);
  Slot* s = sg.s;
  if (!s->stream) HIPCHK(c, hipStreamCreateWithFlags(&s->stream, hipStreamNonBlocking));
  hipStream_t st = s->stream;

  HIPCHK(c, s->A.ensure((size_t)strideA * 8 * chunk));
  HIPCHK(c, s->W.ensure(sizeof(double) * NSB * 256 * (size_t)chunk * nt));
  HIPCHK(c, s->pred_mean.ensure(sizeof(double) * (size_t)m));
  HIPCHK(c, s->map.ensure(sizeof(int32_t) * (size_t)P));
  HIPCHK(c, s->out_lp.ensure(sizeof(double) * (size_t)P));
  HIPCHK(c, s->out_info.ensure(sizeof(int32_t) * (size_t)P));
  PinnedUploads up;
  std::vector<double> noise_sorted, npred;
  if (const int rc = stage_joint(c, s, up, q, pp, chunk, bt, noise_sorted, npred)) return rc;
  if (y_pred) up.add(s->pred_mean.p, y_pred, sizeof(double) * m);
  up.add(s->map.p, bt.order.data(), sizeof(int32_t) * P);
  if (hooks && hooks->stage)
    if (const int rc = hooks->stage(s, up, chunk)) return rc;
  if (!lagr) {
    HIPCHK(c, up.flush(s->h_stage, s->up_blob, st));
  } else if (const int rc = flush_lattice(c, s, st, up, bt, *pl, pl->rank)) {
    return rc;
  }

  for (int p0 = 0; p0 < P; p0 += chunk) {
    const int Pc = std::min(chunk, P - p0);
    launch_init_vec(st, ntot, Pc, s->vec.as<double>(), c->d_xs, (mean_train && n > 0) ? s->mu1.as<double>() : (const double*)nullptr,
                    (int)n, s->info.as<int>() + p0, s->ready.as<int>() + p0);
    if (y_pred)
      launch_init_query_vec(st, Pc, s->vec.as<double>(), ntot, n1_pad, (int)m, s->pred_mean.as<double>(),
                            mean_pred ? s->mu2.as<double>() : (const double*)nullptr);
    CovArgs cv = {};
    cv.tt = s->tt.as<double>(); cv.n1 = (int)n; cv.n1_pad = n1_pad; cv.m2 = (int)m; cv.nt = nt;
    cv.hdr = s->hdr.as<ProgHdr>() + p0; cv.ops = s->ops.as<uint8_t>(); cv.prm = s->prm.as<double>();
    cv.noise = s->noise.as<double>() + p0; cv.noise_q = s->noise_pred.as<double>() + p0;
    cv.A = s->A.as<double>(); cv.strideA = strideA; cv.P = Pc;
    if (lagr) { cv.lagtab = s->lagtab.as<double>(); cv.lagr = s->pl_rank.as<int32_t>(); cv.lag_stride = pl->rank_units * 256; }
    const int nf = std::max(0, std::min(Pc, bt.n_fused - p0));
    const int dcov = nf > 0 ? bt.max_depth_fused : 0;
    cv.p_off = nf;
    HIPCHK(c, launch_cov(st, cv, ntiles, Pc - nf, bt.max_cp, bt.max_depth));

    CholArgs ca = {};
    ca.A = s->A.as<double>(); ca.strideA = strideA; ca.W = s->W.as<double>();
    ca.vec = s->vec.as<double>(); ca.ldv = ntot; ca.partial = s->partial.as<double>();
    ca.info = s->info.as<int>() + p0; ca.P = Pc; ca.nt = nt; ca.k = 0; ca.nt1 = nt;
    set_cov(ca, cv);
    ca.lag = lagr ? 1 : 0;
    ca.n_fused = nf;
    ca.ready = s->ready.as<int>() + p0;
    if (c->flow != 0) {
      if (const int rc = launch_joint_flow(c, s, st, ca, dcov, nt)) return rc;
    } else {
      HIPCHK(c, run_factor(st, ca, nt, dcov, nullptr, nullptr, use_split_diag(c, ca.P)));
    }
    launch_finish_pred_logpdf(st, ca.partial, ca.info, nt1, nt, Pc, (int)m, (int)n, n1_pad, s->map.as<int32_t>() + p0,
                              s->out_lp.as<double>(), s->out_info.as<int32_t>());
    HIPCHK(c, hipGetLastError());
    if (hooks && hooks->chunk)
      if (const int rc = hooks->chunk(s, st, ca, p0, Pc)) return rc;
  }
  std::vector<int32_t> info(P);
  HIPCHK(c, hipStreamSynchronize(st));
  HIPCHK(c, hipMemcpy(out_lp, s->out_lp.p, sizeof(double) * P, hipMemcpyDeviceToHost));
  HIPCHK(c, hipMemcpy(info.data(), s->out_info.p, sizeof(int32_t) * P, hipMemcpyDeviceToHost));
  for (int p = 0; p < P; ++p) {
    if (info[p] < 0) return fail(c, AGP_ERR_HIP, "in-kernel panel solve timed out waiting for its diagonal factor");
    if (out_info) out_info[p] = info[p];
  }
  if (hooks && hooks->done)
    if (const int rc = hooks->done(s)) return rc;
  return AGP_OK;
}

}

namespace {

int toeplitz_predict_sweep(agp_ctx* c, const PredQuery& q, const Particles& pp, int32_t rank0, int mF, const PredLattice& pl,
                           const std::vector<int32_t>& qkind, const std::vector<double>& xq, double* out_mean, double* out_var,
                           int32_t* out_info, const double* xs_sorted_host) {
  HIPCHK(c, hipSetDevice(c->device));
  const int64_t n = q.n, m = q.m;
  const int P = pp.P;
  const double* noise = pp.noise; const double* noise_pred = pp.noise_pred; const double* mean_pred = q.mean_pred;
  Batch bt;
  CompileOpts co;
  co.lag = true; co.lag_units = pl.rank_units; co.rank_extra = 1;
  int rc = compile_batch(c, pp, bt, co);
  if (rc) return rc;
  SlotGuard sg(c);
  Slot* s = sg.s;
  if (!s->stream) HIPCHK(c, hipStreamCreateWithFlags(&s->stream, hipStreamNonBlocking));
  hipStream_t st = s->stream;
// ... 470 lines not shown
    if (!c) return fail(nullptr, AGP_ERR_ARG, "null context");
    if (nq < 0) return fail(c, AGP_ERR_ARG, "negative size");
    if (nq > 0 && !q) return fail(c, AGP_ERR_ARG, "null q");
    for (int64_t k = 0; k < nq; ++k)
      if (!(q[k] > 0.0 && q[k] < 1.0)) return fail(c, AGP_ERR_ARG, "quantile must be in (0, 1)");
    if (const int rc = check_y_transform(c, y_slope, y_intercept)) return rc;
    SumPass sp;
    sp.readout = true; sp.p_rows = p; sp.slope = y_slope; sp.intercept = y_intercept; sp.out_x = out_x;
    sp.z.resize((size_t)nq);
    for (int64_t k = 0; k < nq; ++k) sp.z[(size_t)k] = ndtri(q[k]);
    return sum_batch_body(c, n, ts_pred, p, M, {P, op_off, ops, prm_off, prm, noise, noise_pred}, out_mean, nullptr, nullptr, out_info, &sp);
  });
}

int agp_cov_matrix(agp_ctx* c, const double* ts, int64_t n, const uint8_t* ops, int32_t n_ops, const double* prm,
                   int32_t n_prm, double noise, double* out_K) {
  return abi_guard(c, [&]() -> int {
    if (!c) return fail(nullptr, AGP_ERR_ARG, "null context");
    if (n < 0) return fail(c, AGP_ERR_ARG, "negative size");
    if (n == 0) return AGP_OK;
    if (!ts || !ops || !out_K) return fail(c, AGP_ERR_ARG, "null pointer argument");
    HIPCHK(c, hipSetDevice(c->device));
    const int32_t op_off[2] = {0, n_ops}, prm_off[2] = {0, n_prm};
    double dummy = 0.0;
    Batch bt;
    int rc = compile_batch(c, {1, op_off, ops, prm_off, prm ? prm : &dummy, &noise, nullptr}, bt);
    if (rc) return rc;
    SlotGuard sg(c);
    Slot* s = sg.s;
    if (!s->stream) HIPCHK(c, hipStreamCreateWithFlags(&s->stream, hipStreamNonBlocking));
    hipStream_t st = s->stream;
    const int n_pad = round_up(n, NB), nt = n_pad / NB, ntiles = nt * (nt + 1) / 2;
    const long long strideA = (long long)ntiles * NB2;
    std::vector<double> tt((size_t)n_pad, 0.0);
    std::copy(ts, ts + n, tt.begin());
    HIPCHK(c, s->A.ensure((size_t)strideA * 8));
    HIPCHK(c, s->hdr.ensure(sizeof(ProgHdr)));
    HIPCHK(c, s->ops.ensure(bt.ops.size()));
    HIPCHK(c, s->prm.ensure(sizeof(double) * std::max<size_t>(1, bt.prm.size())));
    HIPCHK(c, s->noise.ensure(sizeof(double)));
    HIPCHK(c, s->tt.ensure(sizeof(double) * (size_t)n_pad));
    HIPCHK(c, s->dense.ensure(sizeof(double) * (size_t)n * n));
    HIPCHK(c, hipMemcpyAsync(s->hdr.p, bt.hdr.data(), sizeof(ProgHdr), hipMemcpyHostToDevice, st));
    HIPCHK(c, hipMemcpyAsync(s->ops.p, bt.ops.data(), bt.ops.size(), hipMemcpyHostToDevice, st));
    if (!bt.prm.empty())
      HIPCHK(c, hipMemcpyAsync(s->prm.p, bt.prm.data(), sizeof(double) * bt.prm.size(), hipMemcpyHostToDevice, st));
    HIPCHK(c, hipMemcpyAsync(s->noise.p, &noise, sizeof(double), hipMemcpyHostToDevice, st));
    HIPCHK(c, hipMemcpyAsync(s->tt.p, tt.data(), sizeof(double) * n_pad, hipMemcpyHostToDevice, st));
    CovArgs cv = {};
    cv.tt = s->tt.as<double>(); cv.n1 = (int)n; cv.n1_pad = n_pad; cv.m2 = 0; cv.nt = nt;
    cv.hdr = s->hdr.as<ProgHdr>(); cv.ops = s->ops.as<uint8_t>(); cv.prm = s->prm.as<double>();
    cv.noise = s->noise.as<double>(); cv.A = s->A.as<double>(); cv.strideA = strideA; cv.P = 1;
    cv.p_off = 0;
    HIPCHK(c, launch_cov(st, cv, ntiles, 1, bt.max_cp, bt.max_depth));
    const long long nel = (long long)n * n;
    launch_unpack_dense(st, s->A.as<double>(), (int)n, 0, s->dense.as<double>());
    HIPCHK(c, hipGetLastError());
    HIPCHK(c, hipMemcpyAsync(out_K, s->dense.p, sizeof(double) * nel, hipMemcpyDeviceToHost, st));
    HIPCHK(c, hipStreamSynchronize(st));
    return AGP_OK;
  });
}

int agp_debug_cholesky(agp_ctx* c, const double* K, int64_t n, double* out_L, int32_t* out_info) {
  if (!c) return fail(nullptr, AGP_ERR_ARG, "null context");
  if (n <= 0 || !K || !out_L) return fail(c, AGP_ERR_ARG, "bad arguments");
  HIPCHK(c, hipSetDevice(c->device));
  SlotGuard sg(c);
  Slot* s = sg.s;
  if (!s->stream) HIPCHK(c, hipStreamCreateWithFlags(&s->stream, hipStreamNonBlocking));
  hipStream_t st = s->stream;
  const int n_pad = round_up(n, NB), nt = n_pad / NB, ntiles = nt * (nt + 1) / 2;
  const long long strideA = (long long)ntiles * NB2;
  const long long nel = (long long)n * n;
  HIPCHK(c, s->A.ensure((size_t)strideA * 8));
  HIPCHK(c, s->W.ensure(sizeof(double) * NSB * 256));
  HIPCHK(c, s->vec.ensure(sizeof(double) * (size_t)n_pad));
  HIPCHK(c, s->partial.ensure(sizeof(double) * 2 * (size_t)nt));
  HIPCHK(c, s->info.ensure(sizeof(int)));
  HIPCHK(c, s->dense.ensure(sizeof(double) * (size_t)nel));
  HIPCHK(c, hipMemcpyAsync(s->dense.p, K, sizeof(double) * nel, hipMemcpyHostToDevice, st));
  HIPCHK(c, hipMemsetAsync(s->vec.p, 0, sizeof(double) * n_pad, st));
  HIPCHK(c, hipMemsetAsync(s->info.p, 0, sizeof(int), st));
  HIPCHK(c, s->ready.ensure(sizeof(int)));
  HIPCHK(c, hipMemsetAsync(s->ready.p, 0, sizeof(int), st));
  launch_pack_dense(st, s->dense.as<double>(), (int)n, nt, strideA, s->A.as<double>());
  CholArgs ca = {};
  ca.A = s->A.as<double>(); ca.strideA = strideA; ca.W = s->W.as<double>(); ca.vec = s->vec.as<double>();
  ca.ldv = n_pad; ca.partial = s->partial.as<double>(); ca.info = s->info.as<int>(); ca.P = 1; ca.nt = nt;
  ca.k = 0; ca.nt1 = nt;
  ca.tt = nullptr; ca.hdr = nullptr; ca.ops = nullptr; ca.prm = nullptr; ca.noise = nullptr; ca.n1 = ca.n1_pad = ca.m2 = 0; ca.n_fused = 0; ca.ready = s->ready.as<int>();
  HIPCHK(c, run_factor(st, ca, nt, 0, nullptr, nullptr, use_split_diag(c, ca.P)));
  launch_unpack_dense(st, s->A.as<double>(), (int)n, 1, s->dense.as<double>());
  HIPCHK(c, hipGetLastError());
  HIPCHK(c, hipMemcpyAsync(out_L, s->dense.p, sizeof(double) * nel, hipMemcpyDeviceToHost, st));
  if (out_info) HIPCHK(c, hipMemcpyAsync(out_info, s->info.p, sizeof(int), hipMemcpyDeviceToHost, st));
  HIPCHK(c, hipStreamSynchronize(st));
  return AGP_OK;
}

int agp_debug_factor_batch(agp_ctx* c, const double* K, const double* y, int64_t n, int32_t P, int32_t schedule,
                           double* out_L, double* out_beta, double* out_partial, int32_t* out_info) {
  if (!c) return fail(nullptr, AGP_ERR_ARG, "null context");
  if (n <= 0 || P <= 0 || !K || !out_L || !out_info) return fail(c, AGP_ERR_ARG, "bad arguments");
  if (schedule < -1 || schedule > 4) return fail(c, AGP_ERR_ARG, "unknown schedule (-1 .. 4)");
  if (n > 8192 || (int64_t)P * n * n > ((int64_t)1 << 28)) return fail(c, AGP_ERR_ARG, "debug probe: batch too large");
  HIPCHK(c, hipSetDevice(c->device));
// ... 255 lines not shown
```

autogp.jl_amd/csrc/agp_store.hip:

```cpp
#include "agp_host.hpp"




constexpr uint64_t STORE_YOUNG_CALLS = 64;
inline size_t store_bytes_per_slot(int nt_cap) {
  const size_t tiles = (size_t)nt_cap * (nt_cap + 1) / 2;
  return tiles * NB2 * 8 + (size_t)nt_cap * NSB * 256 * 8 + (size_t)nt_cap * NB * 8 + (size_t)nt_cap * 2 * 8 + 8;
}

int store_resize(agp_ctx* c, int nt_cap, int n_slots) {
  agp_ctx::FactorStore& fs = c->store;
  if (nt_cap == fs.nt_cap && n_slots == fs.n_slots) return AGP_OK;
  const long long strideA = (long long)nt_cap * (nt_cap + 1) / 2 * NB2;
  const size_t want_bytes = (size_t)n_slots * store_bytes_per_slot(nt_cap);
  if (fs.failed_bytes && want_bytes >= fs.failed_bytes) return fail(c, AGP_ERR_HIP, "factor store: an allocation of this size failed before");
  DevBuf A(Fill::values, &c->poison), W(Fill::values, &c->poison), vec(Fill::values, &c->poison), partial(Fill::values, &c->poison);
  DevBuf info(Fill::never, &c->poison), ready(Fill::never, &c->poison);
  auto bail = [&](hipError_t e, const char* what) {
    A.release(); W.release(); vec.release(); partial.release(); info.release(); ready.release();
    (void)hipGetLastError();
    fs.failed_bytes = want_bytes;
    return fail(c, AGP_ERR_HIP, std::string("factor store: ") + what + ": " + hipGetErrorString(e));
  };
// ... 226 lines not shown
    for (int q = 0; q < U; ++q) { const int u = bt.order[q]; hn[q] = S.noise[u]; hs[q] = slot[u]; hi[q] = i0[u]; }
    std::memcpy(h + o_map, bt.order.data(), sizeof(int32_t) * (size_t)U);
    std::memcpy(h + o_ops, bt.ops.data(), bt.ops.size());
    if (d_out_caller) {
      int32_t* hr = reinterpret_cast<int32_t*>(h + o_rep);
      for (int p = 0; p < P; ++p) hr[p] = rep[p];
    }
    lpl.pack(h);
  }
  char* dstage = static_cast<char*>(s->stage.p);
  EXTCHK(hipMemcpyAsync(dstage, s->h_stage.p, stage_bytes, hipMemcpyHostToDevice, st));
  const int32_t* d_slot = reinterpret_cast<int32_t*>(dstage + o_slot);
  const int32_t* d_i0 = reinterpret_cast<int32_t*>(dstage + o_i0);
  double* d_lp = s->out_lp.as<double>();
  int32_t* d_info = reinterpret_cast<int32_t*>(d_lp + U);

  if (i0min < nt) {
    if (rankm && bt.n_lag_tables > 0) {
      EXTCHK(s->lagtab.ensure(sizeof(double) * (size_t)bt.n_lag_tables * tab_gstride));
      LagArgs la = {};
      la.tt = cltw ? c->d_clt_tt : c->d_ts_lat;
      lpl.point(la, dstage);
      la.tab = s->lagtab.as<double>(); la.nt = cltw ? tab_gstride / NB : (int)((c->n_lat + NB - 1) / NB);
      la.full = 1; la.stride = tab_gstride;
      launch_lag_tables(st, la, tab_gstride / 256, bt.n_lag_tables);
      EXTCHK(hipGetLastError());
    }
    if (c->poison.active()) {
      PoisonRowsArgs pa = {};
      double* bases[4] = {fs.A.as<double>(), fs.W.as<double>(), fs.vec.as<double>(), fs.partial.as<double>()};
      const long long pitch[4] = {fs.strideA, (long long)fs.nt_cap * NSB * 256, (long long)fs.nt_cap * NB, 2LL * fs.nt_cap};
      const long long unit[4] = {NB2, NSB * 256, NB, 2};
      for (int b = 0; b < 4; ++b) { pa.base[b] = bases[b]; pa.pitch[b] = pitch[b]; pa.unit[b] = unit[b]; pa.tri[b] = b == 0; }
      pa.nt_cap = fs.nt_cap; pa.slot = d_slot; pa.i0 = d_i0;
      launch_poison_rows(st, 256, U, 4, pa);
      EXTCHK(hipGetLastError());
      for (int u = 0; u < U; ++u) {
        const long long r0 = std::min<long long>(i0[u], fs.nt_cap);
        c->poison.count(sizeof(double) * (size_t)((fs.strideA - r0 * (r0 + 1) / 2 * NB2) + (fs.nt_cap - r0) * (NSB * 256LL + NB + 2)));
      }
    }
    launch_init_extend(st, U, fs.vec.as<double>(), fs.nt_cap * NB, n_pad, c->d_xs, (int)n, d_slot, d_i0, fs.info.as<int>(), fs.ready.as<int>());
    CovArgs cv = {};
    cv.tt = c->d_ts; cv.n1 = (int)n; cv.n1_pad = n_pad; cv.m2 = 0; cv.nt = nt;
    cv.hdr = reinterpret_cast<ProgHdr*>(dstage + o_hdr); cv.ops = reinterpret_cast<uint8_t*>(dstage + o_ops);
    cv.prm = reinterpret_cast<double*>(dstage + o_prm); cv.noise = reinterpret_cast<double*>(dstage + o_noise);
    cv.A = fs.A.as<double>(); cv.strideA = fs.strideA; cv.P = U; cv.logdt = ge_tab ? c->d_logdt : nullptr;
    cv.lagtab = rankm ? s->lagtab.as<double>() : nullptr; cv.lagr = lagr ? c->d_rank : cltw ? c->d_clt_key : nullptr; cv.lag_stride = tab_units * 256;
    if (cltw) { cv.clt.B = c->d_clt_B; cv.clt.W = 0; cv.clt.nB = clt_nB; cv.clt.gstride = tab_gstride; }
    cv.slot = d_slot; cv.i0 = d_i0;
    const int nf = std::max(0, std::min(U, bt.n_fused));
    const int dcov = nf > 0 ? bt.max_depth_fused : 0;
    cv.p_off = nf;
    EXTCHK(launch_cov(st, cv, nt * (nt + 1) / 2, U - nf, bt.max_cp, bt.max_depth));
    CholArgs ca = {};
    ca.A = cv.A; ca.strideA = fs.strideA; ca.W = fs.W.as<double>(); ca.wsteps = fs.nt_cap;
    ca.vec = fs.vec.as<double>(); ca.ldv = fs.nt_cap * NB; ca.partial = fs.partial.as<double>(); ca.ntp = fs.nt_cap;
    ca.info = fs.info.as<int>(); ca.ready = fs.ready.as<int>(); ca.P = U; ca.nt = nt; ca.k = 0; ca.nt1 = nt;
    set_cov(ca, cv);
    ca.lag = rankm ? 1 : 0;
    ca.n_fused = nf; ca.slot = d_slot; ca.i0 = d_i0;
    if (c->flow > 0 || (c->flow < 0 && U <= FLOW_MAX_PARTICLES && (nt >= 3 || use_flow(c, U, nt)))) {
      const int ntri_cap = fs.nt_cap * (fs.nt_cap + 1) / 2, ntri = nt * (nt + 1) / 2;
      EXTCHK(fs.tflag.ensure(sizeof(int) * (size_t)fs.n_slots * ntri_cap));
      EXTCHK(fs.flowq.ensure(sizeof(int) * 8));
      launch_init_flow_flags(st, U, fs.tflag.as<int>(), ntri_cap, ntri, d_slot, d_i0);
      EXTCHK(hipMemsetAsync(fs.flowq.p, 0, sizeof(int) * 8, st));
      ca.tflag = fs.tflag.as<int>(); ca.ntri = ntri_cap; ca.qnext = fs.flowq.as<int>();
      launch_flow(dcov, 2 * c->n_cu, st, ca);
      EXTCHK(hipGetLastError());
    } else {
      EXTCHK(run_factor_extend(st, ca, dcov, use_split_diag(c, U), i0min));
    }
  }
  launch_finish_logpdf(st, fs.partial.as<double>(), fs.info.as<int>(), nt, U, (int)n, reinterpret_cast<const int*>(dstage + o_map), d_lp, d_info, d_slot, fs.nt_cap);
  EXTCHK(hipGetLastError());
  if (d_out_caller) {
    launch_expand_rep(st, P, d_lp, reinterpret_cast<const int32_t*>(dstage + o_rep), d_out_caller);
    EXTCHK(hipGetLastError());
  }
  EXTCHK(hipMemcpyAsync(s->h_out.p, d_lp, sizeof(double) * U + sizeof(int32_t) * U, hipMemcpyDeviceToHost, st));
  hp_st.stop();
  HostProf hp_w(14);
  EXTCHK(hipStreamSynchronize(st));
  if (d_out_caller && wrote_device) *wrote_device = true;
#undef EXTCHK
  const double* hl = static_cast<const double*>(s->h_out.p);
  const int32_t* hinfo = reinterpret_cast<const int32_t*>(hl + U);
  for (int u = 0; u < U; ++u)
    if (hinfo[u] < 0) { forget_touched(); return fail(c, AGP_ERR_HIP, "in-kernel panel solve timed out waiting for its diagonal factor"); }
  for (int u = 0; u < U; ++u) {
    const int sl = slot[u];
    fs.key[sl] = keys[u]; fs.index[keys[u]] = sl; fs.n_cached[sl] = n; fs.info_h[sl] = hinfo[u];
    if (i0[u] == 0) {
      fs.used[(size_t)sl] = 0; fs.born[(size_t)sl] = call;
      const uint64_t cid = tl_callers ? tl_callers[D.uniq[u]] : 0;
      fs.slot_caller[(size_t)sl] = cid;
      if (cid != 0) {
        auto pr = fs.caller_slot.find(cid);
        if (pr != fs.caller_slot.end() && pr->second != sl && pr->second < fs.n_slots && fs.slot_caller[(size_t)pr->second] == cid &&
            !fs.key[(size_t)pr->second].empty() && fs.used[(size_t)pr->second] == 0)
          fs.used[(size_t)pr->second] = 2;
        fs.caller_slot[cid] = sl;
      }
    }
    if (i0[u] > 0) ++fs.hits; else ++fs.misses;
  }
// ... 210 lines not shown
```

autogp.jl_amd/engine.py:

```python
from __future__ import annotations

import ctypes as C
import os
from pathlib import Path

import numpy as np

from . import gp as _gp

_PKG_DIR = Path(__file__).resolve().parent
LIB_PATH = _PKG_DIR / "lib" / "libautogp_hip.so"

EXPORTED_SYMBOLS = [
    "agp_init", "agp_destroy", "agp_last_error", "agp_version", "agp_set_data", "agp_logpdf",
    "agp_logpdf_batch", "agp_logpdf_grad_batch", "agp_logpdf_grad", "agp_logpdf_batch_device", "agp_predict_batch", "agp_infer_gp_sum", "agp_cov_matrix",
    "agp_debug_cholesky", "agp_debug_mfma_probe", "agp_debug_mfma_peak", "agp_debug_math", "agp_set_profiling", "agp_get_timing", "agp_get_launch_times",
    "agp_set_workspace_limit", "agp_set_coalesce_window", "agp_get_coalesce_stats", "agp_get_dedup_stats",
    "agp_shard_range", "agp_comm_get_unique_id", "agp_comm_init_rank", "agp_comm_info", "agp_init_multi", "agp_set_data_multi",
    "agp_allgather_logweights", "agp_allgather_logweights_device", "agp_logpdf_batch_multi", "agp_logpdf_batch_extend_multi",
    "agp_debug_compact_shards", "agp_logpdf_batch_extend", "agp_extend_stats", "agp_extend_reset", "agp_extend_reserve",
    "agp_predict_reuse_stats", "agp_grad_reuse_stats", "agp_set_factor_cache", "agp_wait", "agp_comm_count", "agp_get_lag_stats", "agp_get_lattice_stats", "agp_get_compact_stats", "agp_set_lattice", "agp_probe_lattice", "agp_set_reference_arithmetic", "agp_shard_plan", "agp_get_coalesce_timing", "agp_set_lag_tables", "agp_set_grad_lag_domain", "agp_get_grad_lag_domain_stats", "agp_get_grad_toeplitz_stats", "agp_get_grad_structured_stats", "agp_get_predict_structured_stats", "agp_get_toeplitz_stats", "agp_set_lag_rank_tables", "agp_get_lag_rank_stats", "agp_get_lag_predict_stats", "agp_get_poison_stats",
    "agp_logpdf_grad_batch_multi", "agp_predict_batch_multi", "agp_extend_stats2", "agp_predict_logpdf_batch",
    "agp_mixture_quantile", "agp_predict_quantile_batch", "agp_infer_gp_sum_batch", "agp_predict_sum_batch",
    "agp_predict_sample_batch", "agp_mixture_moments", "agp_predict_mixture_batch", "agp_get_mixture_stats",
    "agp_remove_data", "agp_get_remove_stats", "agp_set_remove_update", "agp_remove_data_multi",
    "agp_debug_factor_batch", "agp_logpdf_series_batch", "agp_debug_series_factor", "agp_logpdf_grad_series_batch",
]
COMM_ID_BYTES = 128
SERIES_MAX_N = 176


class AGPError(RuntimeError):
    pass


class PosDefException(ArithmeticError):

    def __init__(self, info, particle=None):
        where = "" if particle is None else f" (particle {particle})"
        super().__init__(f"matrix is not positive definite; Cholesky factorization failed at minor {info}{where}")
        self.info = int(info)
        self.particle = particle


_lib = None


def _preload_shared_hip_runtime():
    import importlib.util
    import sys
    if "torch" in sys.modules:
        return
    try:
        spec = importlib.util.find_spec("torch")
        if spec is None or not spec.submodule_search_locations:
            return
        cand = Path(list(spec.submodule_search_locations)[0]) / "lib" / "libamdhip64.so"
        if cand.exists():
            C.CDLL(str(cand), mode=C.RTLD_GLOBAL)
    except Exception:
        pass


def load_library(path=None):
    global _lib
    if _lib is not None and path is None:
        return _lib
    p = Path(path) if path else Path(os.environ.get("AUTOGP_HIP_LIB", LIB_PATH))
    if not p.exists():
        raise AGPError(f"{p} not found: build it with `python -c 'import __graft_entry__ as g; g.build()'` "
                       "(hipcc --offload-arch=gfx950). There is no CPU fallback.")
    _preload_shared_hip_runtime()
    lib = C.CDLL(str(p))
    dp, ip, u8p = C.POINTER(C.c_double), C.POINTER(C.c_int32), C.POINTER(C.c_uint8)
# ... 44 lines not shown
    lib.agp_predict_sum_batch.restype = C.c_int
    lib.agp_cov_matrix.argtypes = [vp, dp, C.c_int64, u8p, C.c_int32, dp, C.c_int32, C.c_double, dp]
    lib.agp_cov_matrix.restype = C.c_int
    lib.agp_debug_cholesky.argtypes = [vp, dp, C.c_int64, dp, ip]; lib.agp_debug_cholesky.restype = C.c_int
    lib.agp_debug_factor_batch.argtypes = [vp, dp, dp, C.c_int64, C.c_int32, C.c_int32, dp, dp, dp, ip]; lib.agp_debug_factor_batch.restype = C.c_int
    lib.agp_debug_series_factor.argtypes = [vp, dp, dp, C.c_int64, C.c_int32, dp, dp, dp, dp, ip]; lib.agp_debug_series_factor.restype = C.c_int
    lib.agp_debug_mfma_probe.argtypes = [vp, dp, dp, dp]; lib.agp_debug_mfma_probe.restype = C.c_int
    lib.agp_debug_mfma_peak.argtypes = [vp, C.c_int32, C.c_int32, dp, dp]; lib.agp_debug_mfma_peak.restype = C.c_int
    lib.agp_debug_math.argtypes = [vp, C.c_int32, dp, dp, dp, C.c_int32]; lib.agp_debug_math.restype = C.c_int
    if hasattr(lib, "agp_debug_gemm_variant"):
        lib.agp_debug_gemm_variant.argtypes = [vp, C.c_int32, C.c_int32, C.c_int32, C.c_int32, C.c_int32, dp]; lib.agp_debug_gemm_variant.restype = C.c_int
    lib.agp_set_profiling.argtypes = [vp, C.c_int]; lib.agp_set_profiling.restype = C.c_int
    lib.agp_get_timing.argtypes = [vp, dp, C.c_int32]; lib.agp_get_timing.restype = C.c_int
    lib.agp_get_launch_times.argtypes = [vp, C.c_int32, dp, C.c_int32]; lib.agp_get_launch_times.restype = C.c_int
    lib.agp_set_workspace_limit.argtypes = [vp, C.c_int64]; lib.agp_set_workspace_limit.restype = C.c_int
    lib.agp_set_coalesce_window.argtypes = [vp, C.c_int32]; lib.agp_set_coalesce_window.restype = C.c_int
    lib.agp_get_coalesce_timing.argtypes = [vp, dp]; lib.agp_get_coalesce_timing.restype = C.c_int
    lib.agp_get_coalesce_stats.argtypes = [vp, C.POINTER(C.c_int64), C.POINTER(C.c_int64)]; lib.agp_get_coalesce_stats.restype = C.c_int
    lib.agp_get_dedup_stats.argtypes = [vp, C.POINTER(C.c_int64), C.POINTER(C.c_int64)]; lib.agp_get_dedup_stats.restype = C.c_int
    lib.agp_get_mixture_stats.argtypes = [vp, C.POINTER(C.c_int64), C.POINTER(C.c_int64)]; lib.agp_get_mixture_stats.restype = C.c_int
    lib.agp_logpdf_batch_extend.argtypes = [vp, C.c_int64, C.c_int32, ip, u8p, ip, dp, dp, dp, ip]
    lib.agp_logpdf_batch_extend.restype = C.c_int
    if hasattr(lib, "agp_debug_flow_trace"):
        lib.agp_debug_flow_trace.argtypes = [vp, C.c_int32, C.c_int64, C.POINTER(C.c_int64)]; lib.agp_debug_flow_trace.restype = C.c_int
    lib.agp_debug_compact_shards.argtypes = [vp, dp, C.c_int32, C.c_int32, dp]; lib.agp_debug_compact_shards.restype = C.c_int
    lib.agp_extend_stats.argtypes = [vp, C.POINTER(C.c_int64)]; lib.agp_extend_stats.restype = C.c_int
    lib.agp_extend_reset.argtypes = [vp, C.c_int]; lib.agp_extend_reset.restype = C.c_int
    lib.agp_extend_stats2.argtypes = [vp, C.POINTER(C.c_int64), C.c_int32]; lib.agp_extend_stats2.restype = C.c_int
    lib.agp_remove_data.argtypes = [vp, C.POINTER(C.c_int64), C.c_int64]; lib.agp_remove_data.restype = C.c_int
    lib.agp_get_remove_stats.argtypes = [vp, C.POINTER(C.c_int64), C.c_int32]; lib.agp_get_remove_stats.restype = C.c_int
    lib.agp_set_remove_update.argtypes = [vp, C.c_int32]; lib.agp_set_remove_update.restype = C.c_int
    lib.agp_remove_data_multi.argtypes = [C.POINTER(vp), C.c_int32, C.POINTER(C.c_int64), C.c_int64]; lib.agp_remove_data_multi.restype = C.c_int
    lib.agp_predict_reuse_stats.argtypes = [vp, C.POINTER(C.c_int64)]; lib.agp_predict_reuse_stats.restype = C.c_int
    lib.agp_grad_reuse_stats.argtypes = [vp, C.POINTER(C.c_int64)]; lib.agp_grad_reuse_stats.restype = C.c_int
    lib.agp_set_factor_cache.argtypes = [vp, C.c_int32]; lib.agp_set_factor_cache.restype = C.c_int
    lib.agp_extend_reserve.argtypes = [vp, C.c_int64, C.c_int32]; lib.agp_extend_reserve.restype = C.c_int
    i32p = C.POINTER(C.c_int32)
    lib.agp_shard_range.argtypes = [C.c_int32, C.c_int32, C.c_int32, i32p, i32p]; lib.agp_shard_range.restype = None
    lib.agp_comm_get_unique_id.argtypes = [vp]; lib.agp_comm_get_unique_id.restype = C.c_int
    lib.agp_comm_init_rank.argtypes = [vp, vp, C.c_int32, C.c_int32]; lib.agp_comm_init_rank.restype = C.c_int
    lib.agp_shard_plan.argtypes = [C.c_int64, C.c_int32, ip, u8p, ip, dp, dp, C.c_int32, C.c_int32, C.c_int64, C.c_int32, i32p, dp, dp]
    lib.agp_shard_plan.restype = C.c_int
    lib.agp_comm_info.argtypes = [vp, i32p, i32p]; lib.agp_comm_info.restype = C.c_int
    lib.agp_comm_count.argtypes = [vp, i32p]; lib.agp_comm_count.restype = C.c_int
    lib.agp_wait.argtypes = [vp]; lib.agp_wait.restype = C.c_int
    lib.agp_get_lag_stats.argtypes = [vp, i32p, C.POINTER(C.c_int64)]; lib.agp_get_lag_stats.restype = C.c_int
    lib.agp_set_lag_tables.argtypes = [vp, C.c_int32]; lib.agp_set_lag_tables.restype = C.c_int
    lib.agp_get_lattice_stats.argtypes = [vp, i32p, C.POINTER(C.c_int64), C.POINTER(C.c_double)]; lib.agp_get_lattice_stats.restype = C.c_int
    lib.agp_get_compact_stats.argtypes = [vp, i32p, C.POINTER(C.c_int64), C.POINTER(C.c_int64)]; lib.agp_get_compact_stats.restype = C.c_int
    lib.agp_set_lattice.argtypes = [vp, C.c_int32]; lib.agp_set_lattice.restype = C.c_int
    lib.agp_get_poison_stats.argtypes = [vp, C.POINTER(C.c_int64), C.POINTER(C.c_int64)]; lib.agp_get_poison_stats.restype = C.c_int
    lib.agp_set_reference_arithmetic.argtypes = [vp, C.c_int32]; lib.agp_set_reference_arithmetic.restype = C.c_int
    lib.agp_probe_lattice.argtypes = [dp, C.c_int64, i32p, C.POINTER(C.c_int64), C.POINTER(C.c_double), C.POINTER(C.c_int64)]; lib.agp_probe_lattice.restype = C.c_int
    lib.agp_set_grad_lag_domain.argtypes = [vp, C.c_int32]; lib.agp_set_grad_lag_domain.restype = C.c_int
    lib.agp_set_lag_rank_tables.argtypes = [vp, C.c_int32]; lib.agp_set_lag_rank_tables.restype = C.c_int
    lib.agp_get_lag_rank_stats.argtypes = [vp, C.POINTER(C.c_int64)]; lib.agp_get_lag_rank_stats.restype = C.c_int
    lib.agp_get_lag_predict_stats.argtypes = [vp, C.POINTER(C.c_int64)]; lib.agp_get_lag_predict_stats.restype = C.c_int
    lib.agp_get_grad_lag_domain_stats.argtypes = [vp, C.POINTER(C.c_int64)]; lib.agp_get_grad_lag_domain_stats.restype = C.c_int
    lib.agp_get_grad_toeplitz_stats.argtypes = [vp, C.POINTER(C.c_int64)]; lib.agp_get_grad_toeplitz_stats.restype = C.c_int
    lib.agp_get_toeplitz_stats.argtypes = [vp, C.POINTER(C.c_int64)]; lib.agp_get_toeplitz_stats.restype = C.c_int
    lib.agp_get_grad_structured_stats.argtypes = [vp, C.POINTER(C.c_int64)]; lib.agp_get_grad_structured_stats.restype = C.c_int
    lib.agp_get_predict_structured_stats.argtypes = [vp, C.POINTER(C.c_int64)]; lib.agp_get_predict_structured_stats.restype = C.c_int
    lib.agp_init_multi.argtypes = [C.POINTER(vp), i32p, C.c_int32]; lib.agp_init_multi.restype = C.c_int
    lib.agp_set_data_multi.argtypes = [C.POINTER(vp), C.c_int32, dp, dp, C.c_int64]; lib.agp_set_data_multi.restype = C.c_int
    lib.agp_allgather_logweights.argtypes = [vp, dp, C.c_int32]; lib.agp_allgather_logweights.restype = C.c_int
    lib.agp_allgather_logweights_device.argtypes = [vp, vp, C.c_int32, vp, vp]; lib.agp_allgather_logweights_device.restype = C.c_int
    lib.agp_logpdf_batch_multi.argtypes = [C.POINTER(vp), C.c_int32, C.c_int64, C.c_int32, ip, u8p, ip, dp, dp, dp, ip]
    lib.agp_logpdf_batch_multi.restype = C.c_int
    lib.agp_logpdf_batch_extend_multi.argtypes = lib.agp_logpdf_batch_multi.argtypes
    lib.agp_logpdf_batch_extend_multi.restype = C.c_int
    lib.agp_logpdf_grad_batch_multi.argtypes = [C.POINTER(vp), C.c_int32, C.c_int64, C.c_int32, ip, u8p, ip, dp, dp, dp, dp, dp, ip, ip]
    lib.agp_logpdf_grad_batch_multi.restype = C.c_int
    lib.agp_predict_batch_multi.argtypes = [C.POINTER(vp), C.c_int32, C.c_int64, dp, C.c_int64, C.c_int32, ip, u8p, ip, dp, dp, dp, dp, dp,
                                            dp, dp, dp, ip, ip]
    lib.agp_predict_batch_multi.restype = C.c_int
    if path is None:
        _lib = lib
    return lib


def _dp(a):
    return a.ctypes.data_as(C.POINTER(C.c_double)) if a is not None else None


def _ip(a):
    return a.ctypes.data_as(C.POINTER(C.c_int32)) if a is not None else None


def _u8(a):
    return a.ctypes.data_as(C.POINTER(C.c_uint8))


def _f64(a):
    return np.ascontiguousarray(np.asarray(a, dtype=np.float64))


def pack_series(series):
    pt_off = np.zeros(len(series) + 1, dtype=np.int64)
    tss, xss = [], []
    for s, (ts, xs) in enumerate(series):
        ts, xs = _f64(ts), _f64(xs)
        if ts.ndim != 1 or xs.ndim != 1:
            raise ValueError(f"series {s}: ts and xs must be vectors")
        if ts.shape != xs.shape:
            raise ValueError(f"series {s}: ts and xs must have equal lengths ({ts.shape[0]} and {xs.shape[0]})")
        if ts.shape[0] > SERIES_MAX_N:
# ... 175 lines not shown
            raise PosDefException(int(info[p]), p)
        return out, info

    def logpdf_grad_series_batch(self, series, nodes, noises, series_index, check=True, programs=None):
        pt_off, ts, xs, (op_off, ops, prm_off, prm), P, noises, sidx = series_call_args(series, nodes, noises, series_index, programs)
        out = np.empty(P, dtype=np.float64); info = np.empty(P, dtype=np.int32); gn = np.empty(P, dtype=np.float64)
        grad = np.zeros(max(1, int(prm_off[-1])))
        ts_arg = ts if ts.size else np.zeros(1)
        xs_arg = xs if xs.size else np.zeros(1)
        prm_arg = prm if prm.size else np.zeros(1)
        self._check(self._lib.agp_logpdf_grad_series_batch(self._ctx, pt_off.shape[0] - 1, pt_off.ctypes.data_as(C.POINTER(C.c_int64)),
                                                           _dp(ts_arg), _dp(xs_arg), P, _ip(sidx), _ip(op_off), _u8(ops), _ip(prm_off),
                                                           _dp(prm_arg), _dp(noises), _dp(out), _dp(grad), _dp(gn), _ip(info)))
        if check and (info > 0).any():
            p = int(np.argmax(info > 0))
            raise PosDefException(int(info[p]), p)
        return out, [grad[prm_off[i]:prm_off[i + 1]] for i in range(P)], gn, info

    def logpdf_batch_extend(self, nodes, noises, n=None, check=True, programs=None):
        n = self.n_max if n is None else int(n)
        op_off, ops, prm_off, prm = programs if programs is not None else _gp.encode_batch(nodes)
        P = op_off.shape[0] - 1
        noises = _f64(noises)
        if noises.shape != (P,):
            raise ValueError("one noise per particle required")
        out = np.empty(P, dtype=np.float64); info = np.empty(P, dtype=np.int32)
        self._check(self._lib.agp_logpdf_batch_extend(self._ctx, n, P, _ip(op_off), _u8(ops), _ip(prm_off), _dp(prm),
                                                      _dp(noises), _dp(out), _ip(info)))
        if check and (info > 0).any():
            p = int(np.argmax(info > 0))
            raise PosDefException(int(info[p]), p)
        return out, info

    def extend_stats(self):
        out = (C.c_int64 * 10)()
        self._check(self._lib.agp_extend_stats2(self._ctx, out, 10))
        return dict(zip(("extended", "from_scratch", "tile_rows_reused", "tile_rows_total", "evicted_before_reuse", "slots", "callers", "occupied",
                         "capacity_tile_rows", "growth_copies"), [int(v) for v in out]))

    def predict_reuse_stats(self):
        out = (C.c_int64 * 2)()
        self._check(self._lib.agp_predict_reuse_stats(self._ctx, out))
        return {"reused": int(out[0]), "factored": int(out[1])}

    def grad_reuse_stats(self):
        out = (C.c_int64 * 2)()
        self._check(self._lib.agp_grad_reuse_stats(self._ctx, out))
        return {"reused": int(out[0]), "factored": int(out[1])}

    def lag_stats(self):
        r = C.c_int32(); k = C.c_int64()
        self._check(self._lib.agp_get_lag_stats(self._ctx, C.byref(r), C.byref(k)))
        return bool(r.value), int(k.value)

    def lattice_stats(self):
        k = C.c_int32(); g = C.c_int64(); h = C.c_double()
        self._check(self._lib.agp_get_lattice_stats(self._ctx, C.byref(k), C.byref(g), C.byref(h)))
        return {"kind": int(k.value), "n_lattice": int(g.value), "spacing": float(h.value)}

    def compact_stats(self):
        w = C.c_int32(); e = C.c_int64(); k = C.c_int64()
        self._check(self._lib.agp_get_compact_stats(self._ctx, C.byref(w), C.byref(e), C.byref(k)))
        return {"lags_per_ordinal": int(w.value), "table_entries": int(e.value), "sweeps": int(k.value)}

    def poison_stats(self):
        b = C.c_int64(); f = C.c_int64()
        self._check(self._lib.agp_get_poison_stats(self._ctx, C.byref(b), C.byref(f)))
        return {"bytes": int(b.value), "fills": int(f.value)}

    def set_lattice(self, on):
        self._check(self._lib.agp_set_lattice(self._ctx, 1 if on else 0))

    def set_reference_arithmetic(self):
        self._check(self._lib.agp_set_reference_arithmetic(self._ctx, 1))

    def set_lag_tables(self, on):
        self._check(self._lib.agp_set_lag_tables(self._ctx, (1 if on else 0) if isinstance(on, bool) else int(on)))

    def set_lag_rank_tables(self, on):
        self._check(self._lib.agp_set_lag_rank_tables(self._ctx, 1 if on else 0))

    def lag_rank_sweeps(self):
        k = C.c_int64()
        self._check(self._lib.agp_get_lag_rank_stats(self._ctx, C.byref(k)))
        return int(k.value)

    def lag_predict_passes(self):
        k = C.c_int64()
        self._check(self._lib.agp_get_lag_predict_stats(self._ctx, C.byref(k)))
        return int(k.value)

    def set_grad_lag_domain(self, on):
        self._check(self._lib.agp_set_grad_lag_domain(self._ctx, (2 if on else 0) if isinstance(on, bool) else int(on)))

    def grad_lag_domain_particles(self):
        k = C.c_int64()
        self._check(self._lib.agp_get_grad_lag_domain_stats(self._ctx, C.byref(k)))
        return int(k.value)

    def toeplitz_particles(self):
        k = C.c_int64()
        self._check(self._lib.agp_get_toeplitz_stats(self._ctx, C.byref(k)))
        return int(k.value)

    def predict_structured_particles(self):
        k = C.c_int64()
# ... 391 lines not shown


def logpdf_grad_batch_multi(engines, nodes, noises, n=None, check=True, programs=None, want_owner=False):
    lib = load_library()
    n = engines[0].n_max if n is None else int(n)
    op_off, ops, prm_off, prm = programs if programs is not None else _gp.encode_batch(nodes)
    P = op_off.shape[0] - 1
    noises = _f64(noises)
    out = np.empty(P); info = np.empty(P, dtype=np.int32); gn = np.empty(P); owner = np.zeros(max(P, 1), dtype=np.int32)
    grad = np.zeros(max(1, int(prm_off[-1])))
    rc = lib.agp_logpdf_grad_batch_multi(_ctx_array(engines), len(engines), n, P, _ip(op_off), _u8(ops), _ip(prm_off), _dp(prm), _dp(noises),
                                         _dp(out), _dp(grad), _dp(gn), _ip(info), _ip(owner))
    engines[0]._check(rc)
    if check and (info > 0).any():
        p = int(np.argmax(info > 0))
        raise PosDefException(int(info[p]), p)
    res = (out, [grad[prm_off[i]:prm_off[i + 1]] for i in range(P)], gn, info)
    return res + (owner[:P],) if want_owner else res


def predict_batch_multi(engines, nodes, noises, ts_pred, n=None, noise_pred=None, mean_train=None, mean_pred=None, want_cov=False,
                        check=True, want_owner=False):
    lib = load_library()
    n = engines[0].n_max if n is None else int(n)
    op_off, ops, prm_off, prm = _gp.encode_batch(nodes)
    P = op_off.shape[0] - 1
    noises = _f64(noises); ts_pred = _f64(ts_pred); m = ts_pred.shape[0]
    npred = None if noise_pred is None else _f64(np.broadcast_to(noise_pred, (P,)))
    mt = None if mean_train is None else _f64(mean_train)
    mp_ = None if mean_pred is None else _f64(mean_pred)
    mean = np.empty((P, m)); var = np.empty((P, m))
    cov = np.empty((P, m, m)) if want_cov else None
    info = np.zeros(P, dtype=np.int32); owner = np.zeros(max(P, 1), dtype=np.int32)
    rc = lib.agp_predict_batch_multi(_ctx_array(engines), len(engines), n, _dp(ts_pred), m, P, _ip(op_off), _u8(ops), _ip(prm_off), _dp(prm),
                                     _dp(noises), _dp(npred), _dp(mt), _dp(mp_), _dp(mean), _dp(var), _dp(cov), _ip(info), _ip(owner))
    engines[0]._check(rc)
    if check and (info > 0).any():
        p = int(np.argmax(info > 0))
        raise PosDefException(int(info[p]), p)
    res = (mean, var, cov, info)
    return res + (owner[:P],) if want_owner else res


def probe_lattice(ts):
    ts = np.ascontiguousarray(ts, dtype=np.float64)
    k = C.c_int32(); g = C.c_int64(); h = C.c_double()
    idx = np.empty(len(ts), dtype=np.int64)
    rc = load_library().agp_probe_lattice(_dp(ts), len(ts), C.byref(k), C.byref(g), C.byref(h), idx.ctypes.data_as(C.POINTER(C.c_int64)))
    if rc != 0:
        raise AGPError(f"agp_probe_lattice failed ({rc})")
    return {"kind": int(k.value), "n_lattice": int(g.value), "spacing": float(h.value), "index": idx}


def _quantile_shape(q, x, conv, iters):
    x, conv, iters = x.T.copy(), conv.T.astype(bool), iters.T.copy()
    if np.ndim(q) == 0:
        return x[:, 0], conv[:, 0], iters[:, 0]
    return x, conv, iters


def raw_components(mean, var, info, n, y_transform=(1.0, 0.0)):
    slope, intercept = (float(v) for v in y_transform)
    mr = (np.asarray(mean, dtype=np.float64) - intercept) / slope
    vr = (1.0 / (slope * slope)) * np.asarray(var, dtype=np.float64)
    info = np.array(info, dtype=np.int32, copy=True)
    bad = ~(np.isfinite(mr) & (vr >= 0.0))
    for p in np.flatnonzero((info == 0) & bad.any(axis=1)):
        info[p] = int(n) + int(np.argmax(bad[p])) + 1
    return mr, vr, info


def predict_quantile_multi(multi, nodes, noises, ts_pred, weights, q, n=None, noise_pred=None, mean_train=None, mean_pred=None,
                           y_transform=(1.0, 0.0), tol=1e-5, max_iter=10**6, check=True):
    engines = multi.engines if isinstance(multi, GPEngineMulti) else list(multi)
    n = engines[0].n_max if n is None else int(n)
    for v in np.atleast_1d(q):
        if not 0.0 < float(v) < 1.0:
            raise AGPError("quantile must be in (0, 1)")
    mean, var, _, info = predict_batch_multi(engines, nodes, noises, ts_pred, n=n, noise_pred=noise_pred, mean_train=mean_train,
                                             mean_pred=mean_pred, check=False)
    mr, vr, info = raw_components(mean, var, info, n, y_transform)
    if check and (info > 0).any():
        p = int(np.argmax(info > 0))
        raise PosDefException(int(info[p]), p)
    if (info != 0).any():
        shape = (len(ts_pred),) + (() if np.ndim(q) == 0 else (len(np.atleast_1d(q)),))
        return np.full(shape, np.nan), np.zeros(shape, dtype=bool), np.zeros(shape, dtype=np.int32), info
    return engines[0].mixture_quantile(mr, vr, weights, q, tol=tol, max_iter=max_iter) + (info,)


class GPEngineMulti:

    def __init__(self, device_ids):
        self._lib = load_library()
        ids = np.ascontiguousarray(np.asarray(device_ids, dtype=np.int32))
        self._n = int(ids.shape[0])
        self._arr = (C.c_void_p * self._n)()
        rc = self._lib.agp_init_multi(self._arr, _ip(ids), self._n)
        if rc != 0:
            msg = self._lib.agp_last_error(None)
            raise AGPError(f"agp_init_multi failed ({rc}): {msg.decode() if msg else ''}")
        self.engines = [GPEngine(int(d), _ctx=C.c_void_p(self._arr[i])) for i, d in enumerate(ids)]
        self.n_max = 0

    def close(self):
        for e in self.engines:
# ... 284 lines not shown
```

include/autogp_hip.h:

```cpp
#ifndef AUTOGP_HIP_H
#define AUTOGP_HIP_H

#include <stdint.h>

#ifdef __cplusplus
extern "C" {
#endif

typedef struct agp_ctx agp_ctx;

#define AGP_OK               0
#define AGP_ERR_ARG         -1
#define AGP_ERR_HIP         -2
#define AGP_ERR_PROGRAM     -3
#define AGP_ERR_NODATA      -4
#define AGP_ERR_COMM        -5
#define AGP_ERR_HOST        -6

#define AGP_MAX_OPS        255

int  agp_init(agp_ctx** out, int device_id);
void agp_destroy(agp_ctx* ctx);
const char* agp_last_error(agp_ctx* ctx);
const char* agp_version(void);

int agp_set_data(agp_ctx* ctx, const double* ts, const double* xs, int64_t n_max);

int agp_logpdf(agp_ctx* ctx, int64_t n,
               const uint8_t* ops, int32_t n_ops, const double* prm, int32_t n_prm,
               double noise, double* out_logpdf, int32_t* out_info);

int agp_logpdf_batch(agp_ctx* ctx, int64_t n, int32_t P,
                     const int32_t* op_off, const uint8_t* ops,
                     const int32_t* prm_off, const double* prm,
                     const double* noise,
                     double* out_logpdf , int32_t* out_info );

#define AGP_SERIES_MAX_N 176
int agp_logpdf_series_batch(agp_ctx* ctx, int32_t S, const int64_t* pt_off , const double* ts, const double* xs,
                            int32_t P, const int32_t* series ,
                            const int32_t* op_off, const uint8_t* ops, const int32_t* prm_off, const double* prm,
                            const double* noise, double* out_logpdf , int32_t* out_info );

int agp_logpdf_grad_series_batch(agp_ctx* ctx, int32_t S, const int64_t* pt_off , const double* ts, const double* xs,
                                 int32_t P, const int32_t* series ,
                                 const int32_t* op_off, const uint8_t* ops, const int32_t* prm_off, const double* prm,
                                 const double* noise,
                                 double* out_logpdf , double* out_grad ,
                                 double* out_grad_noise , int32_t* out_info );

int agp_logpdf_batch_extend(agp_ctx* ctx, int64_t n, int32_t P,
                            const int32_t* op_off, const uint8_t* ops,
                            const int32_t* prm_off, const double* prm,
                            const double* noise,
                            double* out_logpdf , int32_t* out_info );
int agp_extend_stats(agp_ctx* ctx, int64_t* out4);
int agp_extend_stats2(agp_ctx* ctx, int64_t* out, int32_t n_out);
int agp_extend_reset(agp_ctx* ctx, int release_memory);

int agp_remove_data(agp_ctx* ctx, const int64_t* idx, int64_t k);
int agp_get_remove_stats(agp_ctx* ctx, int64_t* out, int32_t n_out);
int agp_set_remove_update(agp_ctx* ctx, int32_t on);
int agp_extend_reserve(agp_ctx* ctx, int64_t n_cap, int32_t n_slots);
int agp_predict_reuse_stats(agp_ctx* ctx, int64_t* out2);
int agp_grad_reuse_stats(agp_ctx* ctx, int64_t* out2);
int agp_set_factor_cache(agp_ctx* ctx, int32_t on);

int agp_get_lag_stats(agp_ctx* ctx, int32_t* regular_grid, int64_t* n_lag_sweeps);
int agp_set_lag_tables(agp_ctx* ctx, int32_t on);

int agp_get_lattice_stats(agp_ctx* ctx, int32_t* kind, int64_t* n_lattice, double* spacing);
int agp_get_compact_stats(agp_ctx* ctx, int32_t* lags_per_ordinal, int64_t* table_entries, int64_t* n_sweeps);
int agp_set_lattice(agp_ctx* ctx, int32_t on);
int agp_get_poison_stats(agp_ctx* ctx, int64_t* bytes, int64_t* fills);
int agp_probe_lattice(const double* ts, int64_t n, int32_t* kind, int64_t* n_lattice, double* spacing, int64_t* index_out);

int agp_set_reference_arithmetic(agp_ctx* ctx, int32_t on);

int agp_get_toeplitz_stats(agp_ctx* ctx, int64_t* n_particles);

int agp_set_lag_rank_tables(agp_ctx* ctx, int32_t on);
int agp_get_lag_rank_stats(agp_ctx* ctx, int64_t* n_sweeps);

int agp_get_lag_predict_stats(agp_ctx* ctx, int64_t* n_passes);
int agp_get_predict_structured_stats(agp_ctx* ctx, int64_t* n_particles);

int agp_set_grad_lag_domain(agp_ctx* ctx, int32_t on);
int agp_get_grad_lag_domain_stats(agp_ctx* ctx, int64_t* n_particles);
int agp_get_grad_toeplitz_stats(agp_ctx* ctx, int64_t* n_particles);
int agp_get_grad_structured_stats(agp_ctx* ctx, int64_t* n_particles);

int agp_logpdf_grad_batch(agp_ctx* ctx, int64_t n, int32_t P,
                          const int32_t* op_off, const uint8_t* ops,
                          const int32_t* prm_off, const double* prm,
                          const double* noise,
                          double* out_logpdf , double* out_grad ,
                          double* out_grad_noise , int32_t* out_info );

int agp_logpdf_grad(agp_ctx* ctx, int64_t n,
                    const uint8_t* ops, int32_t n_ops, const double* prm, int32_t n_prm,
                    double noise, double* out_logpdf, double* out_grad ,
                    double* out_grad_noise, int32_t* out_info);

int agp_logpdf_batch_device(agp_ctx* ctx, int64_t n, int32_t P,
                            const int32_t* op_off, const uint8_t* ops,
                            const int32_t* prm_off, const double* prm,
                            const double* noise,
                            double* d_out_logpdf, int32_t* d_out_info, void* hip_stream);
int agp_wait(agp_ctx* ctx);

int agp_predict_batch(agp_ctx* ctx, int64_t n, const double* ts_pred, int64_t m, int32_t P,
                      const int32_t* op_off, const uint8_t* ops,
                      const int32_t* prm_off, const double* prm,
                      const double* noise, const double* noise_pred,
                      const double* mean_train, const double* mean_pred,
                      double* out_mean, double* out_var, double* out_cov,
                      int32_t* out_info);

int agp_predict_logpdf_batch(agp_ctx* ctx, int64_t n, const double* ts_pred, const double* y_pred, int64_t m, int32_t P,
                             const int32_t* op_off, const uint8_t* ops,
                             const int32_t* prm_off, const double* prm,
                             const double* noise, const double* noise_pred,
                             const double* mean_train, const double* mean_pred,
                             double* out_logpdf, int32_t* out_info);

int agp_mixture_quantile(agp_ctx* ctx, int64_t m, int32_t P, const double* means, const double* vars, const double* weights,
                         const double* q, int64_t nq, double tol, int64_t max_iter, double* out_x, int32_t* out_converged,
                         int32_t* out_iters);
// ... 131 lines not shown
```

Measured before the change: 19880.

## Stage per-node parameter records in LDS and add chain evaluator for covariance

Kernel programs are pre-staged into LDS as fixed 4-double records (three params plus opcode), computed with a wave prefix-sum over parameter counts, so the per-op loop no longer walks a variable parameter offset. Programs whose compiled form is a left-deep chain (leaf, leaf, combine, …) get a flag and are evaluated by a register-only chain evaluator instead of the generic stack machine. The compiler also computes stack need on the compiled tree so lag-table subtrees give a tighter depth. It adds LDS usage sized by max ops, an extra launch argument, and eval stats and probe APIs.

Result: faster. 20220 (median of 6 runs) (+1.7%).

```diff
diff --git a/autogp.jl_amd/__init__.py b/autogp.jl_amd/__init__.py
--- a/autogp.jl_amd/__init__.py
+++ b/autogp.jl_amd/__init__.py
@@ -1,7 +1,7 @@
 from .gp import (Node, LeafNode, BinaryOpNode, WhiteNoise, Constant, Linear, SquaredExponential,
                  GammaExponential, Periodic, Plus, Times, ChangePoint, unroll, encode, encode_batch, from_tuple,
                  split_kernel_sop, extract_kernel)
-from .engine import (GPEngine, GPEngineMulti, shard_range, shard_plan, probe_lattice, logpdf_grad_batch_multi, predict_batch_multi, AGPError, PosDefException, load_library, LIB_PATH, EXPORTED_SYMBOLS,
+from .engine import (GPEngine, GPEngineMulti, shard_range, shard_plan, probe_lattice, probe_program, logpdf_grad_batch_multi, predict_batch_multi, AGPError, PosDefException, load_library, LIB_PATH, EXPORTED_SYMBOLS,
                      compute_cov_matrix_vectorized, eval_cov, mvnormal_logpdf, MvNormal, quantile, infer_gp_sum, predict_proba,
                      predict_quantile, predict_quantile_multi, raw_components, predict_mvn_sum, predict_sum, predict_rand,
                      MixtureModel, predict_mvn, pack_series, series_call_args, SERIES_MAX_N)
diff --git a/autogp.jl_amd/csrc/agp_common.hpp b/autogp.jl_amd/csrc/agp_common.hpp
--- a/autogp.jl_amd/csrc/agp_common.hpp
+++ b/autogp.jl_amd/csrc/agp_common.hpp
@@ -28,6 +28,8 @@
   int32_t lag_off;
 };
 
+constexpr int PROG_CHAIN = 2;
+
 struct LagTabHdr {
   int32_t op_off, n_ops, prm_off, pad_;
 };
diff --git a/autogp.jl_amd/csrc/agp_cov_kernel.hpp b/autogp.jl_amd/csrc/agp_cov_kernel.hpp
--- a/autogp.jl_amd/csrc/agp_cov_kernel.hpp
+++ b/autogp.jl_amd/csrc/agp_cov_kernel.hpp
@@ -13,6 +13,35 @@
          : (o == OP_PLUS || o == OP_TIMES || o == OP_LAG) ? 0 : 3;
 }
 
+constexpr int REC_DOUBLES = 4;
+__device__ __forceinline__ int rec_op(const double* rec, int ip) { return __double2loint(rec[REC_DOUBLES * ip + 3]); }
+__device__ __forceinline__ void stage_node_records(const ProgHdr& h, const uint8_t* __restrict__ ops, const double* __restrict__ prm,
+                                                   double* rec, int tid) {
+  if (tid >= 64) return;
+  int base = 0;
+#pragma unroll
+  for (int i0 = 0; i0 < AGP_MAX_OPS_DEV; i0 += 64) {
+    if (i0 < h.n_ops) {
+      const int i = i0 + tid;
+      const bool live = i < h.n_ops;
+      const int o = live ? (int)ops[i] : OP_PLUS;
+      const int c = prm_count(o);
+      int s = c;
+#pragma unroll
+      for (int d = 1; d < 64; d <<= 1) { const int u = __shfl_up(s, d); if (tid >= d) s += u; }
+      const int q = base + s - c;
+      if (live) {
+        d2 a, b;
+        a.x = c > 0 ? prm[q] : 0.0; a.y = c > 1 ? prm[q + 1] : 0.0;
+        b.x = c > 2 ? prm[q + 2] : 0.0; b.y = __hiloint2double(0, o);
+        *reinterpret_cast<d2*>(rec + REC_DOUBLES * i) = a;
+        *reinterpret_cast<d2*>(rec + REC_DOUBLES * i + 2) = b;
+      }
+      base += __shfl(s, 63);
+    }
+  }
+}
+
 template <bool LAG = false, typename OpT>
 __device__ __forceinline__ void cov_prologue(const double* __restrict__ tt, const uint8_t* __restrict__ code,
                                              int ti, int tj, const ProgHdr& h,
@@ -20,7 +49,8 @@
                                              double* tpt, double* sig, int tid,
                                              const double* __restrict__ lagtab = nullptr, int nt = 0,
                                              const int32_t* __restrict__ rank = nullptr, int lstride = 256, int* xrk = nullptr,
-                                             bool copy_rank_tables = true, const CltArgs clt = CltArgs{}, int* cbl = nullptr) {
+                                             bool copy_rank_tables = true, const CltArgs clt = CltArgs{}, int* cbl = nullptr,
+                                             const double* rec = nullptr) {
   const int g = (tid < NB) ? (ti * NB + tid) : (tj * NB + (tid - NB));
   const double tg = tt[g];
   if (LAG && h.n_lag > 0) {
@@ -52,13 +82,14 @@
     const int cd = code ? (int)code[g] : 0;
     int q = 0, c = 0;
     for (int ip = 0; ip < h.n_ops; ++ip) {
-      const int o = __builtin_amdgcn_readfirstlane((int)ops[ip]);
+      const int o = __builtin_amdgcn_readfirstlane(rec != nullptr ? rec_op(rec, ip) : (int)ops[ip]);
+      const double* pq = rec != nullptr ? rec + REC_DOUBLES * ip : prm + q;
       if (o == OP_CP || o == OP_CP_SWAP) {
-        const double loc = prm[q], sc = prm[q + 1];
+        const double loc = pq[0], sc = pq[1];
         sig[c * 256 + tid] = 0.5 * (1.0 + tanh((loc - t) / sc));
         ++c;
       } else if (o == OP_SEL) {
-        const int id = (int)prm[q];
+        const int id = (int)pq[0];
         sig[c * 256 + tid] = (cd == 0 || cd == id) ? 1.0 : 0.0;
         ++c;
       }
@@ -126,7 +157,28 @@
   }
 }
 
-template <int D, int E, int GEMODE = 0, typename OpT>
+template <int E>
+__device__ __forceinline__ void combine_pair(const int o, const double (&a)[E], double (&b)[E], const double* sg,
+                                             const int (&ri)[E], const int (&ci)[E]) {
+  if (o == OP_PLUS) {
+#pragma unroll
+    for (int e = 0; e < E; ++e) b[e] = a[e] + b[e];
+  } else if (o == OP_TIMES) {
+#pragma unroll
+    for (int e = 0; e < E; ++e) b[e] = a[e] * b[e];
+  } else {
+#pragma unroll
+    for (int e = 0; e < E; ++e) {
+      const double si = sg[ri[e]];
+      const double sj = sg[ci[e]];
+      const double kl = (o == OP_CP) ? a[e] : b[e];
+      const double kr = (o == OP_CP) ? b[e] : a[e];
+      b[e] = (si * sj) * kl + ((1.0 - si) * (1.0 - sj)) * kr;
+    }
+  }
+}
+
+template <int D, int E, int GEMODE = 0, bool REC = false, typename OpT>
 __device__ __forceinline__ void eval_program(const ProgHdr& h, const OpT* __restrict__ ops,
                                              const double* __restrict__ prm, const double* sig,
                                              const double (&tr)[E], const double (&tc)[E],
@@ -141,9 +193,14 @@
 
   int q = 0, cpi = 0, li = 0;
   for (int ip = 0; ip < h.n_ops; ++ip) {
-    const int o = __builtin_amdgcn_readfirstlane((int)ops[ip]);
+    d2 ra = d2{0.0, 0.0}, rb = d2{0.0, 0.0};
+    if (REC) {
+      ra = *reinterpret_cast<const d2*>(prm + REC_DOUBLES * ip);
+      rb = *reinterpret_cast<const d2*>(prm + REC_DOUBLES * ip + 2);
+    }
+    const int o = __builtin_amdgcn_readfirstlane(REC ? __double2loint(rb.y) : (int)ops[ip]);
     if (o <= OP_PER || o >= OP_SEL) {
-      const double p0 = prm[q], p1 = prm[q + 1], p2 = prm[q + 2];
+      const double p0 = REC ? ra.x : prm[q], p1 = REC ? ra.y : prm[q + 1], p2 = REC ? rb.x : prm[q + 2];
       double v[E];
       eval_leaf<E, GEMODE>(o, p0, p1, p2, sig + cpi * 256, lag + li * lstride, tr, tc, ri, ci, lt, etab, v, rk, cb);
       if (o == OP_SEL) ++cpi;
@@ -155,24 +212,8 @@
 #pragma unroll
       for (int e = 0; e < E; ++e) st[0][e] = v[e];
     } else {
-      if (o == OP_PLUS) {
-#pragma unroll
-        for (int e = 0; e < E; ++e) st[0][e] = st[1][e] + st[0][e];
-      } else if (o == OP_TIMES) {
-#pragma unroll
-        for (int e = 0; e < E; ++e) st[0][e] = st[1][e] * st[0][e];
-      } else {
-        const double* sg = sig + cpi * 256;
-#pragma unroll
-        for (int e = 0; e < E; ++e) {
-          const double si = sg[ri[e]];
-          const double sj = sg[ci[e]];
-          const double kl = (o == OP_CP) ? st[1][e] : st[0][e];
-          const double kr = (o == OP_CP) ? st[0][e] : st[1][e];
-          st[0][e] = (si * sj) * kl + ((1.0 - si) * (1.0 - sj)) * kr;
-        }
-        ++cpi;
-      }
+      combine_pair<E>(o, st[1], st[0], sig + cpi * 256, ri, ci);
+      if (o != OP_PLUS && o != OP_TIMES) ++cpi;
 #pragma unroll
       for (int d = 1; d < D - 1; ++d)
 #pragma unroll
@@ -182,6 +223,32 @@
   }
 #pragma unroll
   for (int e = 0; e < E; ++e) out[e] = st[0][e];
+}
+
+template <int E, int GEMODE>
+__device__ __forceinline__ void eval_chain(const ProgHdr& h, const double* __restrict__ rec, const double* sig,
+                                           const double (&tr)[E], const double (&tc)[E],
+                                           const int (&ri)[E], const int (&ci)[E], const double (&lt)[E],
+                                           double (&out)[E], const double* etab, const double* lag,
+                                           const int* rk, int lstride, const int* cb) {
+  int cpi = 0, li = 0;
+  for (int ip = 0; ip < h.n_ops; ip += 2) {
+    const int lp = ip > 0 ? ip - 1 : 0;
+    const d2 ra = *reinterpret_cast<const d2*>(rec + REC_DOUBLES * lp);
+    const d2 rb = *reinterpret_cast<const d2*>(rec + REC_DOUBLES * lp + 2);
+    const int o2 = __builtin_amdgcn_readfirstlane(rec_op(rec, ip));
+    const int o = __builtin_amdgcn_readfirstlane(__double2loint(rb.y));
+    double v[E];
+    eval_leaf<E, GEMODE>(o, ra.x, ra.y, rb.x, sig + cpi * 256, lag + li * lstride, tr, tc, ri, ci, lt, etab, v, rk, cb);
+    if (o == OP_SEL) ++cpi;
+    if (o == OP_LAG) ++li;
+    if (ip > 0) {
+      combine_pair<E>(o2, out, v, sig + cpi * 256, ri, ci);
+      if (o2 != OP_PLUS && o2 != OP_TIMES) ++cpi;
+    }
+#pragma unroll
+    for (int e = 0; e < E; ++e) out[e] = v[e];
+  }
 }
 
 __device__ __forceinline__ double cov_finalize(double v, int gi, int gj, int n1, int n1_pad, int m2, double noise) {
@@ -229,8 +296,10 @@
   const int lstride = rankt ? (a.clt.B != nullptr ? a.clt.gstride : a.lag_stride) : 256;
   int* xrk = reinterpret_cast<int*>(sig + h.n_cp * 256 + (rankt ? 0 : h.n_lag * 256));
   double* etab = reinterpret_cast<double*>(xrk) + (rankt ? 128 : 0);
+  double* rec = etab + AGP_EXP_TAB_N;
   if (AGP_EXP_TABLE && tid < AGP_EXP_TAB_N) etab[tid] = fm::c_exp_tab[tid];
-  cov_prologue<true>(a.tt, a.code, ti, tj, h, ops, prm, tpt, sig, tid, a.lagtab, a.nt, a.lagr, lstride, xrk, false);
+  stage_node_records(h, ops, prm, rec, tid);
+  cov_prologue<true>(a.tt, a.code, ti, tj, h, ops, prm, tpt, sig, tid, a.lagtab, a.nt, a.lagr, lstride, xrk, false, CltArgs{}, nullptr, rec);
   const double* lag = rankt ? a.lagtab + (long long)h.lag_off * lstride : sig + h.n_cp * 256;
   const int* rk = rankt ? xrk : nullptr;
   const int* cb = rankt ? a.clt.B : nullptr;
@@ -252,9 +321,9 @@
 #pragma unroll
     for (int cc = 0; cc < CPP; ++cc) ltn[cc] = *reinterpret_cast<const d2*>(ltile + (long long)(cb0 + cc) * NB + r0);
   }
-  const bool one_node = h.n_ops == 1;
-  const int op1 = one_node ? __builtin_amdgcn_readfirstlane((int)ops[0]) : -1;
-  const double q0 = one_node ? prm[0] : 0.0, q1 = one_node ? prm[1] : 0.0, q2 = one_node ? prm[2] : 0.0;
+  const bool one_node = h.n_ops == 1, chain = (h.flags & PROG_CHAIN) != 0;
+  const int op1 = one_node ? __builtin_amdgcn_readfirstlane(rec_op(rec, 0)) : -1;
+  const double q0 = one_node ? rec[0] : 0.0, q1 = one_node ? rec[1] : 0.0, q2 = one_node ? rec[2] : 0.0;
   for (int pass = 0; pass < NPASS; ++pass) {
     const int c0 = cb0 + pass * CPP;
     double tr[E], tc[E], out[E], lt[E];
@@ -273,7 +342,8 @@
       ci[e] = NB + c0 + (e >> 1);
     }
     if (one_node) eval_leaf<E, 0>(op1, q0, q1, q2, sig, lag, tr, tc, ri, ci, lt, etab, out, rk, cb);
-    else eval_program<D, E, 0>(h, ops, prm, sig, tr, tc, ri, ci, lt, out, etab, lag, rk, lstride, cb);
+    else if (D <= 4 && chain) eval_chain<E, 0>(h, rec, sig, tr, tc, ri, ci, lt, out, etab, lag, rk, lstride, cb);
+    else eval_program<D, E, 0, true>(h, ops, rec, sig, tr, tc, ri, ci, lt, out, etab, lag, rk, lstride, cb);
 #pragma unroll
     for (int cc = 0; cc < CPP; ++cc) {
       const int gj = tj * NB + c0 + cc;
diff --git a/autogp.jl_amd/csrc/agp_engine.hip b/autogp.jl_amd/csrc/agp_engine.hip
--- a/autogp.jl_amd/csrc/agp_engine.hip
+++ b/autogp.jl_amd/csrc/agp_engine.hip
@@ -155,7 +155,7 @@
 }
 
 void emit(const std::vector<CNode>& nodes, int id, Compiled& out, bool ge_tab, bool lag = false,
-          const std::vector<char>* stat = nullptr, const std::vector<char>* heavy = nullptr) {
+          const std::vector<char>* stat = nullptr, const std::vector<char>* heavy = nullptr, const std::vector<int>* cneed = nullptr) {
   const CNode& nd = nodes[id];
   if (lag && stat && (*stat)[id] && (*heavy)[id]) {
     Compiled sub;
@@ -191,9 +191,9 @@
     }
     return;
   }
-  const bool swap = nodes[nd.right].need > nodes[nd.left].need;
-  emit(nodes, swap ? nd.right : nd.left, out, ge_tab, lag, stat, heavy);
-  emit(nodes, swap ? nd.left : nd.right, out, ge_tab, lag, stat, heavy);
+  const bool swap = cneed ? (*cneed)[nd.right] > (*cneed)[nd.left] : nodes[nd.right].need > nodes[nd.left].need;
+  emit(nodes, swap ? nd.right : nd.left, out, ge_tab, lag, stat, heavy, cneed);
+  emit(nodes, swap ? nd.left : nd.right, out, ge_tab, lag, stat, heavy, cneed);
   if (nd.op == OP_CP) {
     out.ops.push_back((uint8_t)(swap ? OP_CP_SWAP : OP_CP));
     out.prm.push_back(nd.prm[0]);
@@ -202,6 +202,21 @@
   } else {
     out.ops.push_back((uint8_t)nd.op);
   }
+}
+
+int compiled_need(const std::vector<CNode>& nodes, int id, const std::vector<char>& stat, const std::vector<char>& heavy, std::vector<int>& cneed) {
+  const CNode& nd = nodes[id];
+  if (nd.left < 0 || (stat[id] && heavy[id])) return cneed[id] = 1;
+  const int a = compiled_need(nodes, nd.left, stat, heavy, cneed), b = compiled_need(nodes, nd.right, stat, heavy, cneed);
+  return cneed[id] = (a == b) ? a + 1 : std::max(a, b);
+}
+
+bool is_chain(const std::vector<uint8_t>& ops) {
+  auto leaf = [](int o) { return o <= OP_PER || o >= OP_SEL; };
+  if (ops.empty() || ops.size() % 2 == 0 || !leaf(ops[0])) return false;
+  for (size_t i = 1; i + 1 < ops.size(); i += 2)
+    if (!leaf(ops[i]) || leaf(ops[i + 1])) return false;
+  return true;
 }
 
 const char* compile_program(const uint8_t* ops, int n_ops, const double* prm, int n_prm, Compiled& out,
@@ -244,11 +259,14 @@
   if (lag) {
     std::vector<char> stat(nodes.size(), 0), heavy(nodes.size(), 0);
     classify(nodes, stack[0], stat, heavy);
-    emit(nodes, stack[0], out, false, true, &stat, &heavy);
+    std::vector<int> cneed(nodes.size(), 1);
+    const int need_c = compiled_need(nodes, stack[0], stat, heavy, cneed);
+    emit(nodes, stack[0], out, false, true, &stat, &heavy, &cneed);
+    out.depth_need = need_c;
     if (out.n_cp + out.n_lag > COV_MAX_TABLES) {
       Compiled plain;
       emit(nodes, stack[0], plain, false, false);
-      plain.depth_need = out.depth_need;
+      plain.depth_need = nodes[stack[0]].need;
       out = plain;
     }
   } else {
@@ -328,7 +346,8 @@
     h.n_ops = (int32_t)cp.ops.size();
     h.n_cp = cp.n_cp;
     h.n_prm = (int32_t)cp.prm.size();
-    h.flags = cp.uses_tab ? 1 : 0;
+    const bool chain = is_chain(cp.ops);
+    h.flags = (cp.uses_tab ? 1 : 0) | (chain ? PROG_CHAIN : 0);
     h.n_lag = cp.n_lag; h.lag_off = bt.n_lag_tables;
     bt.n_lag_tables += cp.n_lag;
     for (LagTabHdr th : cp.thdr) {
@@ -343,12 +362,16 @@
     const int lds_units = cp.n_cp + cp.n_lag * o.lag_units + o.rank_extra;
     bt.max_cp = std::max(bt.max_cp, o.rank_extra > 0 ? cp.n_cp + 1 : lds_units);
     bt.max_depth = std::max(bt.max_depth, cp.depth_need);
+    bt.max_ops = std::max(bt.max_ops, (int)cp.ops.size());
+    if (!fusable(bt.order[q])) { ++bt.n_eval[3]; if (chain && cp.ops.size() > 1) ++bt.n_eval[4]; }
+    else ++bt.n_eval[cp.ops.size() == 1 ? 0 : 2];
     if (fusable(bt.order[q])) {
       bt.n_fused = q + 1;
       bt.max_cp_fused = std::max(bt.max_cp_fused, lds_units);
       bt.max_depth_fused = std::max(bt.max_depth_fused, cp.depth_need);
     }
   }
+  if (bt.max_depth > 4) bt.n_eval[4] = 0;
   if (o.want_grad) {
     bt.ghdr.resize(P);
     for (int q = 0; q < P; ++q) {
@@ -854,6 +877,7 @@
   if (go && bt.g_max_nodes > 64) return fail(c, AGP_ERR_PROGRAM, "gradient supports kernel trees of up to 64 nodes");
   if (go && n > 23040) return fail(c, AGP_ERR_ARG, "gradient sweeps address a particle's packed matrix with 32-bit byte offsets: n <= 23040");
   if (lag) { std::lock_guard<std::mutex> g(c->mu); ++c->n_lag_sweeps; }
+  { std::lock_guard<std::mutex> g(c->mu); for (int i = 0; i < 5; ++i) c->eval_stats[i] = bt.n_eval[i]; }
   int32_t toep_rank0 = 0;
   bool any_toep_sweep = false;
   std::vector<int32_t> toep_retry;
@@ -1143,7 +1167,7 @@
         const int dcov = nf > 0 ? bt.max_depth_fused : 0;
         size_t e0 = pf.mark(q);
         cv.p_off = nf;
-        if (!(n_hit > 0 && i0min == nt)) HIPCHK(c, launch_cov(q, cv, ntiles, Pg - nf, bt.max_cp, bt.max_depth));
+        if (!(n_hit > 0 && i0min == nt)) HIPCHK(c, launch_cov(q, cv, ntiles, Pg - nf, bt.max_cp, bt.max_depth, bt.max_ops));
         size_t e1 = pf.mark(q);
         pf.span(1, e0, e1);
 
@@ -1657,6 +1681,29 @@
   return cf;
 }
 
+int agp_probe_program(const uint8_t* ops, int32_t n_ops, const double* prm, int32_t n_prm, int32_t* n_compiled, int32_t* chain,
+                      int32_t* depth, int32_t* n_tables) {
+  if (!ops || (n_prm > 0 && !prm)) return AGP_ERR_ARG;
+  try {
+    Compiled cp;
+    if (compile_program(ops, n_ops, prm, n_prm, cp, false, false, true)) return AGP_ERR_PROGRAM;
+    if (n_compiled) *n_compiled = (int32_t)cp.ops.size();
+    if (chain) *chain = is_chain(cp.ops) ? 1 : 0;
+    if (depth) *depth = cp.depth_need;
+    if (n_tables) *n_tables = cp.n_lag;
+  } catch (const std::exception&) {
+    return AGP_ERR_ARG;
+  }
+  return AGP_OK;
+}
+
+int agp_get_eval_stats(agp_ctx* c, int64_t* out5) {
+  if (!c || !out5) return fail(c, AGP_ERR_ARG, "null pointer");
+  std::lock_guard<std::mutex> g(c->mu);
+  for (int i = 0; i < 5; ++i) out5[i] = c->eval_stats[i];
+  return AGP_OK;
+}
+
 int agp_probe_lattice(const double* ts, int64_t n, int32_t* kind, int64_t* n_lattice, double* spacing, int64_t* index_out) {
   if (n < 0 || (n > 0 && !ts)) return AGP_ERR_ARG;
   for (int64_t i = 0; i < n; ++i)
diff --git a/autogp.jl_amd/csrc/agp_host.hpp b/autogp.jl_amd/csrc/agp_host.hpp
--- a/autogp.jl_amd/csrc/agp_host.hpp
+++ b/autogp.jl_amd/csrc/agp_host.hpp
@@ -273,6 +273,7 @@
   int lag_enable = 1;
   double lag_tol_h = 1e-11;
   int64_t n_lag_sweeps = 0;
+  int64_t eval_stats[5] = {0, 0, 0, 0, 0};
   double* d_logdt = nullptr;
   size_t logdt_cap = 0;
   bool logdt_ok = false;
@@ -386,7 +387,9 @@
   int n_fused = 0;
   int max_cp = 0;
   int max_depth = 1;
+  int max_ops = 1;
   int max_cp_fused = 0, max_depth_fused = 1;
+  int64_t n_eval[5] = {0, 0, 0, 0, 0};
   int n_lag_tables = 0;
   std::vector<LagTabHdr> thdr;
   std::vector<uint8_t> tops;
diff --git a/autogp.jl_amd/csrc/agp_kernels.hip b/autogp.jl_amd/csrc/agp_kernels.hip
--- a/autogp.jl_amd/csrc/agp_kernels.hip
+++ b/autogp.jl_amd/csrc/agp_kernels.hip
@@ -37,9 +37,11 @@
   return hipSuccess;
 }
 
-hipError_t launch_cov(hipStream_t st, const CovArgs& ca, int ntiles, int P, int max_cp, int depth) {
+hipError_t launch_cov(hipStream_t st, const CovArgs& ca, int ntiles, int P, int max_cp, int depth, int max_ops) {
   if (ntiles <= 0 || P <= 0) return hipSuccess;
-  const size_t lds = (256 + (size_t)max_cp * 256 + AGP_EXP_TAB_N) * sizeof(double);
+  if (max_ops < 1 || max_ops > AGP_MAX_OPS_DEV) return hipErrorInvalidValue;
+  const size_t lds = (256 + (size_t)max_cp * 256 + AGP_EXP_TAB_N + (size_t)REC_DOUBLES * max_ops) * sizeof(double);
+  if (lds > (size_t)DYN_LDS_MAX_BYTES_K) return hipErrorInvalidValue;
   CovArgs cs = ca;
   cs.csplit = ((long long)ntiles * P < 4096) ? 4 : 1;
   dim3 grid(ntiles, P, cs.csplit), block(256);
diff --git a/autogp.jl_amd/csrc/agp_launch.hpp b/autogp.jl_amd/csrc/agp_launch.hpp
--- a/autogp.jl_amd/csrc/agp_launch.hpp
+++ b/autogp.jl_amd/csrc/agp_launch.hpp
@@ -4,7 +4,7 @@
 namespace agp {
 
 hipError_t kernels_init();
-hipError_t launch_cov(hipStream_t st, const CovArgs& ca, int ntiles, int P, int max_cp, int depth);
+hipError_t launch_cov(hipStream_t st, const CovArgs& ca, int ntiles, int P, int max_cp, int depth, int max_ops);
 void launch_lag_tables(hipStream_t st, const LagArgs& la, int units, int n_tables);
 hipError_t launch_toep_logpdf(hipStream_t st, const ToepArgs& ta);
 void launch_logdt_tiles(hipStream_t st, unsigned ntiles, const double* ts, double* out);
diff --git a/autogp.jl_amd/csrc/agp_predict.hip b/autogp.jl_amd/csrc/agp_predict.hip
--- a/autogp.jl_amd/csrc/agp_predict.hip
+++ b/autogp.jl_amd/csrc/agp_predict.hip
@@ -317,7 +317,7 @@
     cv.p_off = nf;
     cv.skip_pred_offdiag = want_cov ? 0 : 1;
     cv.i0 = n_hit > 0 ? d_i0 + p0 : nullptr;
-    HIPCHK(c, launch_cov(st, cv, ntiles, Pc - nf, bt.max_cp, bt.max_depth));
+    HIPCHK(c, launch_cov(st, cv, ntiles, Pc - nf, bt.max_cp, bt.max_depth, bt.max_ops));
 
     CholArgs ca = {};
     ca.A = s->A.as<double>(); ca.strideA = strideA; ca.W = s->W.as<double>();
@@ -387,7 +387,7 @@
       if (lagr && nf > 0) {
         CovArgs cp = cv;
         cp.p_off = 0; cp.pred_only = 1; cp.i0 = nullptr;
-        HIPCHK(c, launch_cov(st, cp, ntiles, nf, bt.max_cp, bt.max_depth));
+        HIPCHK(c, launch_cov(st, cp, ntiles, nf, bt.max_cp, bt.max_depth, bt.max_ops));
         ca.n_fused = 0; dcov_s = 0;
       }
       launch_update_schur(dcov_s, 8 * Pg * T, st, ca);
@@ -521,7 +521,7 @@
     const int nf = std::max(0, std::min(Pc, bt.n_fused - p0));
     const int dcov = nf > 0 ? bt.max_depth_fused : 0;
     cv.p_off = nf;
-    HIPCHK(c, launch_cov(st, cv, ntiles, Pc - nf, bt.max_cp, bt.max_depth));
+    HIPCHK(c, launch_cov(st, cv, ntiles, Pc - nf, bt.max_cp, bt.max_depth, bt.max_ops));
 
     CholArgs ca = {};
     ca.A = s->A.as<double>(); ca.strideA = strideA; ca.W = s->W.as<double>();
@@ -1098,7 +1098,7 @@
     cv.hdr = s->hdr.as<ProgHdr>(); cv.ops = s->ops.as<uint8_t>(); cv.prm = s->prm.as<double>();
     cv.noise = s->noise.as<double>(); cv.A = s->A.as<double>(); cv.strideA = strideA; cv.P = 1;
     cv.p_off = 0;
-    HIPCHK(c, launch_cov(st, cv, ntiles, 1, bt.max_cp, bt.max_depth));
+    HIPCHK(c, launch_cov(st, cv, ntiles, 1, bt.max_cp, bt.max_depth, bt.max_ops));
     const long long nel = (long long)n * n;
     launch_unpack_dense(st, s->A.as<double>(), (int)n, 0, s->dense.as<double>());
     HIPCHK(c, hipGetLastError());
diff --git a/autogp.jl_amd/csrc/agp_store.hip b/autogp.jl_amd/csrc/agp_store.hip
--- a/autogp.jl_amd/csrc/agp_store.hip
+++ b/autogp.jl_amd/csrc/agp_store.hip
@@ -302,7 +302,7 @@
     const int nf = std::max(0, std::min(U, bt.n_fused));
     const int dcov = nf > 0 ? bt.max_depth_fused : 0;
     cv.p_off = nf;
-    EXTCHK(launch_cov(st, cv, nt * (nt + 1) / 2, U - nf, bt.max_cp, bt.max_depth));
+    EXTCHK(launch_cov(st, cv, nt * (nt + 1) / 2, U - nf, bt.max_cp, bt.max_depth, bt.max_ops));
     CholArgs ca = {};
     ca.A = cv.A; ca.strideA = fs.strideA; ca.W = fs.W.as<double>(); ca.wsteps = fs.nt_cap;
     ca.vec = fs.vec.as<double>(); ca.ldv = fs.nt_cap * NB; ca.partial = fs.partial.as<double>(); ca.ntp = fs.nt_cap;
diff --git a/autogp.jl_amd/engine.py b/autogp.jl_amd/engine.py
--- a/autogp.jl_amd/engine.py
+++ b/autogp.jl_amd/engine.py
@@ -19,7 +19,7 @@
     "agp_shard_range", "agp_comm_get_unique_id", "agp_comm_init_rank", "agp_comm_info", "agp_init_multi", "agp_set_data_multi",
     "agp_allgather_logweights", "agp_allgather_logweights_device", "agp_logpdf_batch_multi", "agp_logpdf_batch_extend_multi",
     "agp_debug_compact_shards", "agp_logpdf_batch_extend", "agp_extend_stats", "agp_extend_reset", "agp_extend_reserve",
-    "agp_predict_reuse_stats", "agp_grad_reuse_stats", "agp_set_factor_cache", "agp_wait", "agp_comm_count", "agp_get_lag_stats", "agp_get_lattice_stats", "agp_get_compact_stats", "agp_set_lattice", "agp_probe_lattice", "agp_set_reference_arithmetic", "agp_shard_plan", "agp_get_coalesce_timing", "agp_set_lag_tables", "agp_set_grad_lag_domain", "agp_get_grad_lag_domain_stats", "agp_get_grad_toeplitz_stats", "agp_get_grad_structured_stats", "agp_get_predict_structured_stats", "agp_get_toeplitz_stats", "agp_set_lag_rank_tables", "agp_get_lag_rank_stats", "agp_get_lag_predict_stats", "agp_get_poison_stats",
+    "agp_predict_reuse_stats", "agp_grad_reuse_stats", "agp_set_factor_cache", "agp_wait", "agp_comm_count", "agp_get_lag_stats", "agp_get_lattice_stats", "agp_get_compact_stats", "agp_set_lattice", "agp_probe_lattice", "agp_probe_program", "agp_get_eval_stats", "agp_set_reference_arithmetic", "agp_shard_plan", "agp_get_coalesce_timing", "agp_set_lag_tables", "agp_set_grad_lag_domain", "agp_get_grad_lag_domain_stats", "agp_get_grad_toeplitz_stats", "agp_get_grad_structured_stats", "agp_get_predict_structured_stats", "agp_get_toeplitz_stats", "agp_set_lag_rank_tables", "agp_get_lag_rank_stats", "agp_get_lag_predict_stats", "agp_get_poison_stats",
     "agp_logpdf_grad_batch_multi", "agp_predict_batch_multi", "agp_extend_stats2", "agp_predict_logpdf_batch",
     "agp_mixture_quantile", "agp_predict_quantile_batch", "agp_infer_gp_sum_batch", "agp_predict_sum_batch",
     "agp_predict_sample_batch", "agp_mixture_moments", "agp_predict_mixture_batch", "agp_get_mixture_stats",
@@ -170,6 +170,8 @@
     lib.agp_get_poison_stats.argtypes = [vp, C.POINTER(C.c_int64), C.POINTER(C.c_int64)]; lib.agp_get_poison_stats.restype = C.c_int
     lib.agp_set_reference_arithmetic.argtypes = [vp, C.c_int32]; lib.agp_set_reference_arithmetic.restype = C.c_int
     lib.agp_probe_lattice.argtypes = [dp, C.c_int64, i32p, C.POINTER(C.c_int64), C.POINTER(C.c_double), C.POINTER(C.c_int64)]; lib.agp_probe_lattice.restype = C.c_int
+    lib.agp_probe_program.argtypes = [C.POINTER(C.c_uint8), C.c_int32, dp, C.c_int32, i32p, i32p, i32p, i32p]; lib.agp_probe_program.restype = C.c_int
+    lib.agp_get_eval_stats.argtypes = [C.c_void_p, C.POINTER(C.c_int64)]; lib.agp_get_eval_stats.restype = C.c_int
     lib.agp_set_grad_lag_domain.argtypes = [vp, C.c_int32]; lib.agp_set_grad_lag_domain.restype = C.c_int
     lib.agp_set_lag_rank_tables.argtypes = [vp, C.c_int32]; lib.agp_set_lag_rank_tables.restype = C.c_int
     lib.agp_get_lag_rank_stats.argtypes = [vp, C.POINTER(C.c_int64)]; lib.agp_get_lag_rank_stats.restype = C.c_int
@@ -451,6 +453,11 @@
         r = C.c_int32(); k = C.c_int64()
         self._check(self._lib.agp_get_lag_stats(self._ctx, C.byref(r), C.byref(k)))
         return bool(r.value), int(k.value)
+
+    def eval_stats(self):
+        out = (C.c_int64 * 5)()
+        self._check(self._lib.agp_get_eval_stats(self._ctx, out))
+        return dict(zip(("one_node", "chain", "stack", "prebuilt", "prebuilt_chain"), (int(v) for v in out)))
 
     def lattice_stats(self):
         k = C.c_int32(); g = C.c_int64(); h = C.c_double()
@@ -948,6 +955,16 @@
     return {"kind": int(k.value), "n_lattice": int(g.value), "spacing": float(h.value), "index": idx}
 
 
+def probe_program(node):
+    ops, prm = _gp.encode(node)
+    prm_arg = prm if prm.size else np.zeros(1)
+    n = C.c_int32(); ch = C.c_int32(); d = C.c_int32(); nt = C.c_int32()
+    rc = load_library().agp_probe_program(_u8(ops), ops.size, _dp(prm_arg), prm.size, C.byref(n), C.byref(ch), C.byref(d), C.byref(nt))
+    if rc != 0:
+        raise AGPError(f"agp_probe_program failed ({rc})")
+    return {"n_compiled": int(n.value), "chain": bool(ch.value), "depth": int(d.value), "n_tables": int(nt.value)}
+
+
 def _quantile_shape(q, x, conv, iters):
     x, conv, iters = x.T.copy(), conv.T.astype(bool), iters.T.copy()
     if np.ndim(q) == 0:
diff --git a/include/autogp_hip.h b/include/autogp_hip.h
--- a/include/autogp_hip.h
+++ b/include/autogp_hip.h
@@ -74,6 +74,9 @@
 int agp_set_lattice(agp_ctx* ctx, int32_t on);
 int agp_get_poison_stats(agp_ctx* ctx, int64_t* bytes, int64_t* fills);
 int agp_probe_lattice(const double* ts, int64_t n, int32_t* kind, int64_t* n_lattice, double* spacing, int64_t* index_out);
+int agp_probe_program(const uint8_t* ops, int32_t n_ops, const double* prm, int32_t n_prm, int32_t* n_compiled, int32_t* chain,
+                      int32_t* depth, int32_t* n_tables);
+int agp_get_eval_stats(agp_ctx* ctx, int64_t* out5);
 
 int agp_set_reference_arithmetic(agp_ctx* ctx, int32_t on);
 
```
